# rustformers/llm

Measured on AMD Instinct MI355X. Metric: decode tokens/s LLaMA-7B Q4_0, higher is better.
Workload: dtype i8*i4->i32 block dots, f32 accumulate (W4A8 = ggml's Q4_0·Q8_0)

## Files before the change

### include/ggml_hip.h

```cpp
#ifndef GGML_HIP_H
#define GGML_HIP_H

#include <stdbool.h>
#include <stddef.h>
#include <stdint.h>

#ifdef __cplusplus
extern "C" {
#endif

#define GGML_API __attribute__((visibility("default")))

#define GGML_FILE_MAGIC 0x67676d6c
#define GGML_FILE_VERSION 1
#define GGML_QNT_VERSION 2
#define GGML_QNT_VERSION_FACTOR 1000
#define GGML_MAX_DIMS 4
#define GGML_MAX_NODES 4096
#define GGML_MAX_PARAMS 256
#define GGML_MAX_CONTEXTS 64
#define GGML_MAX_SRC 6
#define GGML_MAX_NAME 48
#define GGML_MAX_OP_PARAMS 32
#define GGML_DEFAULT_N_THREADS 4
// ... 307 lines not shown
GGML_API struct ggml_tensor *ggml_soft_max(struct ggml_context *ctx, struct ggml_tensor *a);
GGML_API struct ggml_tensor *ggml_soft_max_inplace(struct ggml_context *ctx, struct ggml_tensor *a);
GGML_API struct ggml_tensor *ggml_rope(struct ggml_context *ctx, struct ggml_tensor *a, int n_past, int n_dims,
                                       int mode, int n_ctx);
GGML_API struct ggml_tensor *ggml_rope_inplace(struct ggml_context *ctx, struct ggml_tensor *a, int n_past,
                                               int n_dims, int mode, int n_ctx);
GGML_API struct ggml_tensor *ggml_rope_custom_inplace(struct ggml_context *ctx, struct ggml_tensor *a,
                                                      int n_past, int n_dims, int mode, int n_ctx,
                                                      float freq_base, float freq_scale);
GGML_API struct ggml_tensor *ggml_alibi(struct ggml_context *ctx, struct ggml_tensor *a, int n_past, int n_head,
                                        float bias_max);
GGML_API struct ggml_tensor *ggml_flash_attn(struct ggml_context *ctx, struct ggml_tensor *q,
                                             struct ggml_tensor *k, struct ggml_tensor *v, bool masked);
GGML_API struct ggml_tensor *ggml_map_unary_f32(struct ggml_context *ctx, struct ggml_tensor *a,
                                                ggml_unary_op_f32_t fun);
GGML_API struct ggml_tensor *ggml_map_binary_f32(struct ggml_context *ctx, struct ggml_tensor *a,
                                                 struct ggml_tensor *b, ggml_binary_op_f32_t fun);

GGML_API struct ggml_cgraph *ggml_new_graph(struct ggml_context *ctx);
GGML_API size_t ggml_graph_overhead(void);
GGML_API void ggml_build_forward_expand(struct ggml_cgraph *cgraph, struct ggml_tensor *tensor);
GGML_API struct ggml_cgraph ggml_build_forward(struct ggml_tensor *tensor);
GGML_API struct ggml_cplan ggml_graph_plan(struct ggml_cgraph *cgraph, int n_threads);
GGML_API int ggml_graph_compute(struct ggml_cgraph *cgraph, struct ggml_cplan *cplan);
GGML_API void ggml_graph_reset(struct ggml_cgraph *cgraph);

GGML_API size_t ggml_quantize_q4_0(const float *src, void *dst, int n, int k, int64_t *hist);
GGML_API size_t ggml_quantize_q4_1(const float *src, void *dst, int n, int k, int64_t *hist);
GGML_API size_t ggml_quantize_q5_0(const float *src, void *dst, int n, int k, int64_t *hist);
GGML_API size_t ggml_quantize_q5_1(const float *src, void *dst, int n, int k, int64_t *hist);
GGML_API size_t ggml_quantize_q8_0(const float *src, void *dst, int n, int k, int64_t *hist);
GGML_API size_t ggml_quantize_q2_K(const float *src, void *dst, int n, int k, int64_t *hist);
GGML_API size_t ggml_quantize_q3_K(const float *src, void *dst, int n, int k, int64_t *hist);
GGML_API size_t ggml_quantize_q4_K(const float *src, void *dst, int n, int k, int64_t *hist);
GGML_API size_t ggml_quantize_q5_K(const float *src, void *dst, int n, int k, int64_t *hist);
GGML_API size_t ggml_quantize_q6_K(const float *src, void *dst, int n, int k, int64_t *hist);
GGML_API size_t ggml_quantize_chunk(enum ggml_type type, const float *src, void *dst, int start, int n,
                                    int64_t *hist);
GGML_API ggml_type_traits_t ggml_internal_get_type_traits(enum ggml_type i);

GGML_API int ggml_cpu_has_blas(void);
GGML_API int ggml_cpu_has_gpublas(void);

#define GGML_HIP_MAX_DEVICES 16

GGML_API void ggml_init_hipblas(void);
GGML_API void ggml_hip_set_tensor_split(const float *tensor_split);
GGML_API void ggml_hip_mul(const struct ggml_tensor *src0, const struct ggml_tensor *src1,
                           struct ggml_tensor *dst);
GGML_API bool ggml_hip_can_mul_mat(const struct ggml_tensor *src0, const struct ggml_tensor *src1,
                                   struct ggml_tensor *dst);
GGML_API size_t ggml_hip_mul_mat_get_wsize(const struct ggml_tensor *src0, const struct ggml_tensor *src1,
                                           struct ggml_tensor *dst);
GGML_API void ggml_hip_mul_mat(const struct ggml_tensor *src0, const struct ggml_tensor *src1,
                               struct ggml_tensor *dst, void *wdata, size_t wsize);
GGML_API void *ggml_hip_host_malloc(size_t size);
GGML_API void ggml_hip_host_free(void *ptr);
GGML_API void ggml_hip_transform_tensor(void *data, struct ggml_tensor *tensor);
GGML_API void ggml_hip_free_data(struct ggml_tensor *tensor);
GGML_API void ggml_hip_assign_buffers(struct ggml_tensor *tensor);
GGML_API void ggml_hip_assign_buffers_no_scratch(struct ggml_tensor *tensor);
GGML_API void ggml_hip_assign_buffers_force_inplace(struct ggml_tensor *tensor);
GGML_API void ggml_hip_set_main_device(int main_device);
GGML_API void ggml_hip_set_mul_mat_q(bool mul_mat_q);
GGML_API void ggml_hip_set_scratch_size(size_t scratch_size);
GGML_API void ggml_hip_free_scratch(void);
GGML_API bool ggml_hip_compute_forward(struct ggml_compute_params *params, struct ggml_tensor *tensor);

GGML_API void ggml_init_cublas(void);
GGML_API void ggml_cuda_set_tensor_split(const float *tensor_split);
GGML_API void ggml_cuda_mul(const struct ggml_tensor *, const struct ggml_tensor *, struct ggml_tensor *);
GGML_API bool ggml_cuda_can_mul_mat(const struct ggml_tensor *, const struct ggml_tensor *, struct ggml_tensor *);
GGML_API size_t ggml_cuda_mul_mat_get_wsize(const struct ggml_tensor *, const struct ggml_tensor *,
                                            struct ggml_tensor *);
GGML_API void ggml_cuda_mul_mat(const struct ggml_tensor *, const struct ggml_tensor *, struct ggml_tensor *,
                                void *, size_t);
GGML_API void *ggml_cuda_host_malloc(size_t size);
GGML_API void ggml_cuda_host_free(void *ptr);
GGML_API void ggml_cuda_transform_tensor(void *data, struct ggml_tensor *tensor);
GGML_API void ggml_cuda_free_data(struct ggml_tensor *tensor);
GGML_API void ggml_cuda_assign_buffers(struct ggml_tensor *tensor);
GGML_API void ggml_cuda_assign_buffers_no_scratch(struct ggml_tensor *tensor);
GGML_API void ggml_cuda_assign_buffers_force_inplace(struct ggml_tensor *tensor);
GGML_API void ggml_cuda_set_main_device(int main_device);
GGML_API void ggml_cuda_set_mul_mat_q(bool mul_mat_q);
GGML_API void ggml_cuda_set_scratch_size(size_t scratch_size);
GGML_API void ggml_cuda_free_scratch(void);
GGML_API bool ggml_cuda_compute_forward(struct ggml_compute_params *params, struct ggml_tensor *tensor);

GGML_API int ggml_hip_device_count(void);
GGML_API int ggml_hip_slot_physical_device(int slot);
GGML_API int ggml_hip_thread_session_slot(void);
GGML_API int ggml_hip_get_main_device(void);
GGML_API void ggml_hip_bind_thread_device(int device);
GGML_API int ggml_hip_thread_pinned_device(void);
GGML_API void ggml_hip_unbind_thread_device(void);
GGML_API int ggml_hip_get_tensor_split(float *out, int cap);
GGML_API void ggml_hip_set_layer_split(const float *fractions, int n);
GGML_API int ggml_hip_get_layer_split(float *out, int cap);
GGML_API void ggml_hip_copy_between_devices(int dst_device, void *dst, int src_device, const void *src, size_t nbytes);
GGML_API void ggml_hip_synchronize(void);
GGML_API void ggml_hip_tensor_get(const struct ggml_tensor *tensor, void *host_dst, size_t offset, size_t nbytes);
GGML_API void ggml_hip_tensor_set(struct ggml_tensor *tensor, const void *host_src, size_t offset, size_t nbytes);
GGML_API void ggml_hip_memcpy(void *dst, const void *src, size_t nbytes, int kind);
GGML_API void *ggml_hip_tensor_device_ptr(const struct ggml_tensor *tensor);
enum ggml_hip_kclass {
    GGML_HIP_KCLASS_MMVQ = 0,
    GGML_HIP_KCLASS_MMQ_MFMA,
    GGML_HIP_KCLASS_ATTN,
    GGML_HIP_KCLASS_OTHER,
    GGML_HIP_KCLASS_COUNT
};
GGML_API void ggml_hip_timing_begin(void);
GGML_API void ggml_hip_timing_end(void);
GGML_API void ggml_hip_timing_query(int kclass, double *ms, int64_t *launches, double *algo_bytes);
GGML_API void ggml_hip_set_option(const char *key, int value);
GGML_API int ggml_hip_get_option(const char *key);
#define GGML_HIP_KKIND_BASE 16
GGML_API int ggml_hip_bench_plan_class(int kclass, int replays, double *ms_total, int64_t *launches_per_replay,
                                       double *algo_bytes_per_replay);
#define GGML_HIP_COMM_ID_BYTES 128
GGML_API int ggml_hip_comm_unique_id(void *id_out );
GGML_API int ggml_hip_comm_init(int rank, int world, const void *id);
GGML_API void ggml_hip_comm_destroy(void);
GGML_API int ggml_hip_comm_ranks(void);
GGML_API void ggml_hip_comm_send(const void *dev_src, size_t nbytes, int peer);
GGML_API void ggml_hip_comm_recv(void *dev_dst, size_t nbytes, int peer);
GGML_API void ggml_hip_comm_sendrecv(const void *dev_src, int send_peer, void *dev_dst, int recv_peer, size_t nbytes);
GGML_API int ggml_hip_bench_empty(int wgs, int threads, int lds_bytes, int kernarg_bytes, int n_launch, int replays,
                                  double *out);
GGML_API int64_t ggml_hip_get_stat(const char *key);
GGML_API int ggml_hip_graph_compute_begin(struct ggml_cgraph *cgraph);
GGML_API void ggml_hip_graph_compute_end(void);
GGML_API int ggml_hip_graph_prepare(struct ggml_cgraph *cgraph);
GGML_API void ggml_hip_expect_greedy_next(void);
GGML_API int ggml_hip_decode_greedy_chain(struct ggml_cgraph *last, int n, int32_t *out_tokens, float *last_logits);
GGML_API int ggml_hip_decode_batch(struct ggml_cgraph *const *graphs, int n_graphs);
GGML_API int ggml_hip_decode_batch_greedy(struct ggml_cgraph *const *graphs, int n_graphs, int n_steps, int32_t *out_ids);
GGML_API int ggml_hip_topk(const struct ggml_tensor *t, int64_t row, int k, const int32_t *extra_ids, int n_extra,
                           float *out_vals, int32_t *out_ids);
GGML_API int ggml_hip_row_probs(const struct ggml_tensor *logits, int64_t row_begin, int64_t n_rows, const int32_t *targets,
                                float *out_probs);
GGML_API size_t ggml_hip_quantize(enum ggml_type type, const float *src, void *dst, int64_t n, int64_t k, int64_t *hist);
GGML_API int ggml_hip_quantize_resident(const struct ggml_tensor *src, struct ggml_tensor *dst, int64_t *hist);
GGML_API size_t ggml_hip_read_timeline(int64_t *dst, size_t max_records);
GGML_API int ggml_hip_debug_prompt_attention(const float *q, const uint16_t *mem_k, const uint16_t *mem_v, float *out, int N, int E,
                                             int Egqa, int H, int n_past, int64_t C, float scale, int fused);
GGML_API int ggml_hip_debug_prompt_attention_plan(const float *q_raw, const float *q_raw2, const float *rope, const uint16_t *mem_k,
                                                  const uint16_t *mem_v, uint16_t *x16, float *out, int N, int E, int Egqa, int H,
                                                  int n_past, int64_t C, float scale, int f16d);
GGML_API int ggml_hip_debug_exp_le0(uint16_t *out_fast, uint16_t *out_ref);
GGML_API int ggml_hip_debug_token_tail(const float *logits, int V, const float *emb, int E, int n_past, int misalign,
                                       int32_t *id_tail, int32_t *id_argmax, float *slot_logits, float *slot_emb, int32_t *prm_out);
GGML_API int ggml_hip_debug_batch_tail(const float *logits, int B, int V, const int32_t *pos_in, const int32_t *tokens_in,
                                       int32_t *ids_out, int32_t *prm_out, int32_t *pos_out);
GGML_API int ggml_hip_debug_mul_mat_cols(const struct ggml_tensor *w, const float *x, float *out, int N);
GGML_API int ggml_hip_debug_mat_vec_big(const struct ggml_tensor *w0, const struct ggml_tensor *w1, const struct ggml_tensor *w2,
                                        int xsrc, int epi, const float *x, const float *norm_w, float eps, const float *res, float *out,
                                        float *y_out, int n_past, int D, float freq_base, float freq_scale, int64_t C,
                                        uint16_t *mem_k, uint16_t *mem_v);
GGML_API int ggml_hip_debug_mat_vec_kbig(const struct ggml_tensor *w0, const struct ggml_tensor *w1, const struct ggml_tensor *w2,
                                         int xsrc, int epi, const float *x, const float *xw, float eps, const float *res, float *out,
                                         float *y_out, int n_past, int D, float freq_base, float freq_scale, int64_t C,
                                         uint16_t *mem_k, uint16_t *mem_v);
GGML_API int ggml_hip_debug_mat_vec_f16(const struct ggml_tensor *w0, const struct ggml_tensor *w1, const struct ggml_tensor *w2,
                                        int xsrc, int epi, const float *x, const float *xw, float eps, const float *res, float *out,
                                        float *y_out, int n_past, int D, float freq_base, float freq_scale, int64_t C,
                                        uint16_t *mem_k, uint16_t *mem_v, int ncols);
GGML_API int ggml_hip_share_stream(int slot, int with_slot);
GGML_API const char *ggml_hip_version(void);

#ifdef __cplusplus
}
#endif

#ifdef __cplusplus
#define GGML_ABI_ASSERT(c, m) static_assert(c, m)
#else
#define GGML_ABI_ASSERT(c, m) _Static_assert(c, m)
#endif
GGML_ABI_ASSERT(sizeof(struct ggml_object) == 32, "ggml_object size (lib.rs:239)");
GGML_ABI_ASSERT(offsetof(struct ggml_object, type) == 24, "ggml_object.type");
GGML_ABI_ASSERT(sizeof(struct ggml_tensor) == 272, "ggml_tensor size (lib.rs:446)");
GGML_ABI_ASSERT(offsetof(struct ggml_tensor, ne) == 16, "ggml_tensor.ne");
GGML_ABI_ASSERT(offsetof(struct ggml_tensor, nb) == 48, "ggml_tensor.nb");
GGML_ABI_ASSERT(offsetof(struct ggml_tensor, op) == 80, "ggml_tensor.op");
GGML_ABI_ASSERT(offsetof(struct ggml_tensor, op_params) == 84, "ggml_tensor.op_params");
GGML_ABI_ASSERT(offsetof(struct ggml_tensor, is_param) == 116, "ggml_tensor.is_param");
GGML_ABI_ASSERT(offsetof(struct ggml_tensor, grad) == 120, "ggml_tensor.grad");
GGML_ABI_ASSERT(offsetof(struct ggml_tensor, src) == 128, "ggml_tensor.src");
GGML_ABI_ASSERT(offsetof(struct ggml_tensor, perf_runs) == 176, "ggml_tensor.perf_runs");
GGML_ABI_ASSERT(offsetof(struct ggml_tensor, data) == 200, "ggml_tensor.data");
GGML_ABI_ASSERT(offsetof(struct ggml_tensor, name) == 208, "ggml_tensor.name");
GGML_ABI_ASSERT(offsetof(struct ggml_tensor, extra) == 256, "ggml_tensor.extra");
GGML_ABI_ASSERT(offsetof(struct ggml_tensor, padding) == 264, "ggml_tensor.padding");
GGML_ABI_ASSERT(sizeof(struct ggml_cplan) == 16424, "ggml_cplan size");
GGML_ABI_ASSERT(offsetof(struct ggml_cplan, n_tasks) == 20, "ggml_cplan.n_tasks");
GGML_ABI_ASSERT(offsetof(struct ggml_cplan, abort_callback) == 16408, "ggml_cplan.abort_callback");
GGML_ABI_ASSERT(sizeof(struct ggml_cgraph) == 164520, "ggml_cgraph size (lib.rs:651)");
GGML_ABI_ASSERT(offsetof(struct ggml_cgraph, nodes) == 8, "ggml_cgraph.nodes");
GGML_ABI_ASSERT(offsetof(struct ggml_cgraph, leafs) == 65544, "ggml_cgraph.leafs");
GGML_ABI_ASSERT(offsetof(struct ggml_cgraph, visited_hash_table) == 98312, "ggml_cgraph.visited_hash_table");
GGML_ABI_ASSERT(offsetof(struct ggml_cgraph, perf_runs) == 164496, "ggml_cgraph.perf_runs");
GGML_ABI_ASSERT(sizeof(struct ggml_scratch) == 24, "ggml_scratch size");
GGML_ABI_ASSERT(sizeof(struct ggml_init_params) == 24, "ggml_init_params size");
GGML_ABI_ASSERT(sizeof(struct ggml_compute_params) == 32, "ggml_compute_params size");
GGML_ABI_ASSERT(offsetof(struct ggml_compute_params, wsize) == 16, "ggml_compute_params.wsize");
GGML_ABI_ASSERT(sizeof(ggml_type_traits_t) == 40, "ggml_type_traits_t size");

#endif
```

### llm_amd/csrc/backend_state.inc

```

[[noreturn]] void die(const char *fmt, ...) {
    char buf[1024];
    va_list ap;
    va_start(ap, fmt);
    vsnprintf(buf, sizeof(buf), fmt, ap);
    va_end(ap);
    fatal_note("%s", buf);
    abort();
}

int g_cur_slot();
struct Arena {
    uintptr_t base = 0;
    size_t size = 0;
    char *dev = nullptr;
    bool live = true;
    bool is_scratch = false;
};

struct DevTensor {
    uint32_t magic = 0x48495054;
    int slot = (int)(g_cur_slot());
    uintptr_t host = 0;
    size_t nbytes = 0;
    char *dev = nullptr;
    size_t dev_bytes = 0;
    bool soa = false;
    bool auto_uploaded = false;
    int refs = 1;
    bool zero_filled = false;
    uintptr_t owner_hdr = 0;
    QWeight qw{};
    char *w16 = nullptr;
    size_t w16_size = 0;
    bool ksoa = false;
    KWeight kw{};
    ggml_type type = GGML_TYPE_F32;
    int64_t ne[4] = {0, 0, 0, 0};
};

struct Timing {
    bool on = false;
    struct Rec {
        hipEvent_t a, b;
    };
    std::vector<Rec> recs[GGML_HIP_KCLASS_COUNT];
    std::vector<Rec> pool;
    double bytes[GGML_HIP_KCLASS_COUNT] = {0, 0, 0, 0};
    int64_t launches[GGML_HIP_KCLASS_COUNT] = {0, 0, 0, 0};
};

#define GGML_HIP_MAX_BACKENDS 16
struct Backend {
    int slot = 0;
    bool inited = false;
    int device = 0;
    hipStream_t stream = nullptr;
    hipStream_t own_stream = nullptr;
    std::recursive_mutex mu;
    hipEvent_t xfer_ev = nullptr;
    int opt_fuse_heads = 1, opt_attn_one = 1, opt_attn_split = 1;
    std::map<uintptr_t, Arena> arenas;
    std::map<uintptr_t, DevTensor *> tensors;
    std::map<uintptr_t, DevTensor *> auto_tensors;
    struct WsChunk {
        char *p;
        size_t size;
    };
    std::vector<WsChunk> ws_chunks;
    size_t ws_off = 0;
    Timing timing;
    int opt_fuse = 1, opt_plan = 1, opt_plan_k = 1, opt_plan_multi = 1, opt_plan_prompt = 1, opt_graph = 1, opt_big = 1, opt_kbig = 1;
    int opt_chain_k = 0, opt_prepare = 1, opt_plan_batch = 1, opt_plan_f16 = 1, opt_plan_batch_chain = 1;
    int opt_fuse_attn = 1, opt_fuse_wo = 1, opt_warm_mb = 24, opt_affine = 1;
    int opt_act_quant = 0, opt_mmq_i8 = 0;
    int opt_mmq_min = 32, opt_k_prompt_min = 12, opt_mmq_fuse = 3, opt_mmq_cols = 1, opt_mmq_t256 = 1, opt_attn_fused = 1;
    int opt_mmq_w16 = 1, opt_w16_headroom_gb = 16;
    int opt_probe = 0;
    std::atomic<size_t> w16_bytes{0};
    uint64_t w16_gen = 1;
    int num_cus = 256;
    long long *timeline = nullptr;
    size_t timeline_bytes = 0;
    int timeline_wgs = 4;
    uint64_t stat_plan_tokens = 0, stat_generic_graphs = 0, stat_split_tokens = 0, stat_prompt_plan_tokens = 0, stat_fused_tokens = 0, stat_kplan_tokens = 0, stat_fused_heads_tokens = 0, stat_fused_wo_tokens = 0, stat_fused_affine_tokens = 0, stat_prepared_tokens = 0;
    uint64_t stat_alibi_fused = 0;
    uint64_t stat_batch_tokens = 0, stat_batch_steps = 0, stat_batch_chain_steps = 0, stat_batch_chain_tokens = 0;
    uint64_t stat_flash_attn_nodes = 0;
    enum { MMQ_K_PLAIN, MMQ_K_DMA_P8, MMQ_K_W16_P8, MMQ_K_W16_256, MMQ_K_I8, MMQ_K_COUNT };
    uint64_t stat_mmq[MMQ_K_COUNT] = {0, 0, 0, 0, 0};
    void *chain_plan = nullptr;
    ggml_cgraph *chain_graph = nullptr;
    bool pending_wait = false;
    bool pending_light = false;
    int opt_speculate_next = 0, opt_token_tail = 1;
    bool greedy_hint = false;
    struct Spec {
        bool pending = false;
        void *plan = nullptr;
        int n_past = 0, av = 0;
        int parity = 0;
        int32_t fed_id = 0;
        bool fed_id_valid = false;
        int cooldown = 0;
    } spec;
    struct TailWait {
        void *plan = nullptr;
        int q = 0;
        void *logits_dst = nullptr, *emb_dst = nullptr;
        bool staged = false;
    } tail;
    void *res_plan = nullptr;
    uint64_t stat_tail_tokens = 0, stat_result_copies = 0, stat_tail_hits = 0, stat_tail_misses = 0;
    uint64_t stat_spec_hits = 0, stat_spec_misses = 0;
    unsigned *ferr_pin = nullptr;
    void *ferr_plan = nullptr;
    int opt_fused_fallback = 1, opt_fused_rearm_tokens = 256;
    uint64_t fused_rearm_at = 0;
    uint64_t fused_rearm_stretch = 0;
    int fused_saved_fuse_attn = 0, fused_saved_attn_one = 0;
    uint64_t stat_fused_rearms = 0;
    uint64_t stat_cols_warm_launches = 0;
    int opt_test_fused_timeout = 0;
    uint64_t stat_fused_timeouts = 0;
    uint64_t ns_match = 0, ns_launch = 0, ns_wait = 0, ns_compute = 0, ns_mirror = 0, stat_mirror_bytes = 0;
    size_t dead_shadow_bytes = 0;
    uint64_t arena_seen = 0;
    void *prep = nullptr;
    int opt_gen = 0;
    int xcd_labels = -1;
    void *hot_line = nullptr;
    int session_records = 0;
};
enum : unsigned {
    OPT_ENV = 1,
    OPT_DROPS = 2,
    OPT_DEVICE = 4,
    OPT_ACTION = 8,
};
enum OptEffect { FX_NONE, FX_ACT_QUANT, FX_TIMELINE, FX_MMQ_W16, FX_W16_RELEASE, FX_FUSE_ATTN, FX_SPECULATE_NEXT, FX_FUSED_REARM_TOKENS, FX_TEST_FUSED_TIMEOUT, FX_SERIAL_STAGE_SLOTS };
struct OptRow {
    const char *key;
    int Backend::*field;
    unsigned flags;
    OptEffect fx = FX_NONE;
    int lo = 0, hi = -1;
};
static const OptRow g_options[] = {
    {"fuse", &Backend::opt_fuse, OPT_ENV},
    {"plan", &Backend::opt_plan, OPT_ENV},
    {"plan_k", &Backend::opt_plan_k, OPT_ENV | OPT_DROPS},
    {"plan_f16", &Backend::opt_plan_f16, OPT_ENV | OPT_DROPS},
    {"plan_multi", &Backend::opt_plan_multi, OPT_ENV | OPT_DROPS},
    {"plan_prompt", &Backend::opt_plan_prompt, OPT_ENV | OPT_DROPS},
    {"plan_batch", &Backend::opt_plan_batch, OPT_ENV | OPT_DROPS},
    {"plan_batch_chain", &Backend::opt_plan_batch_chain, OPT_ENV},
    {"graph", &Backend::opt_graph, OPT_ENV},
    {"big", &Backend::opt_big, OPT_ENV | OPT_DROPS},
    {"kbig", &Backend::opt_kbig, OPT_ENV | OPT_DROPS},
    {"chain_k", &Backend::opt_chain_k, OPT_ENV, FX_NONE, 0, 64},
    {"prepare", &Backend::opt_prepare, OPT_ENV},
    {"speculate_next", &Backend::opt_speculate_next, OPT_ENV, FX_SPECULATE_NEXT},
    {"token_tail", &Backend::opt_token_tail, OPT_ENV, FX_SPECULATE_NEXT},
    {"fuse_attn", &Backend::opt_fuse_attn, OPT_ENV | OPT_DROPS, FX_FUSE_ATTN},
    {"fuse_wo", &Backend::opt_fuse_wo, OPT_ENV | OPT_DROPS},
    {"warm_mb", &Backend::opt_warm_mb, OPT_ENV | OPT_DROPS},
    {"affine", &Backend::opt_affine, OPT_ENV | OPT_DROPS},
    {"fuse_heads", &Backend::opt_fuse_heads, OPT_ENV | OPT_DROPS},
    {"attn_split", &Backend::opt_attn_split, OPT_ENV | OPT_DROPS},
    {"attn_one", &Backend::opt_attn_one, OPT_ENV | OPT_DROPS},
    {"fused_fallback", &Backend::opt_fused_fallback, OPT_ENV},
    {"fused_rearm_tokens", &Backend::opt_fused_rearm_tokens, OPT_ENV, FX_FUSED_REARM_TOKENS},
    {"act_quant", &Backend::opt_act_quant, OPT_ENV | OPT_DEVICE, FX_ACT_QUANT},
    {"mmq_i8", &Backend::opt_mmq_i8, OPT_ENV},
    {"mmq_min", &Backend::opt_mmq_min, OPT_ENV},
    {"k_prompt_min", &Backend::opt_k_prompt_min, OPT_ENV},
    {"mmq_fuse", &Backend::opt_mmq_fuse, OPT_ENV},
    {"mmq_cols", &Backend::opt_mmq_cols, OPT_ENV | OPT_DROPS},
    {"mmq_t256", &Backend::opt_mmq_t256, OPT_ENV | OPT_DROPS},
    {"attn_fused", &Backend::opt_attn_fused, OPT_ENV},
    {"mmq_w16", &Backend::opt_mmq_w16, OPT_ENV | OPT_DROPS | OPT_DEVICE, FX_MMQ_W16},
    {"w16_headroom_gb", &Backend::opt_w16_headroom_gb, OPT_ENV},
    {"w16_release", nullptr, OPT_DEVICE | OPT_ACTION, FX_W16_RELEASE},
    {"serial_stage_slots", nullptr, 0, FX_SERIAL_STAGE_SLOTS},
    {"timeline", nullptr, OPT_DEVICE, FX_TIMELINE},
    {"probe", &Backend::opt_probe, OPT_DROPS},
    {"test_fused_timeout", &Backend::opt_test_fused_timeout, OPT_DROPS, FX_TEST_FUSED_TIMEOUT},
};
const OptRow &opt_row(const char *key, const char *who) {
    for (const OptRow &o : g_options)
        if (!strcmp(o.key, key)) return o;
    die("%s: unknown key '%s'", who, key);
}
inline int opt_value(const OptRow &o, int v) {
    if (o.fx == FX_ACT_QUANT) return v ? 1 : 0;
    return o.lo <= o.hi ? std::min(o.hi, std::max(o.lo, v)) : v;
}
struct StatRow {
    const char *key;
    uint64_t Backend::*field;
};
static const StatRow g_counters[] = {
    {"plan_tokens", &Backend::stat_plan_tokens},
    {"fused_attn_tokens", &Backend::stat_fused_tokens},
    {"fused_heads_tokens", &Backend::stat_fused_heads_tokens},
    {"fused_wo_tokens", &Backend::stat_fused_wo_tokens},
    {"fused_affine_tokens", &Backend::stat_fused_affine_tokens},
    {"attn_split_tokens", &Backend::stat_split_tokens},
    {"kplan_tokens", &Backend::stat_kplan_tokens},
    {"prepared_tokens", &Backend::stat_prepared_tokens},
    {"prompt_plan_tokens", &Backend::stat_prompt_plan_tokens},
    {"batch_decode_tokens", &Backend::stat_batch_tokens},
    {"batch_decode_steps", &Backend::stat_batch_steps},
    {"batch_chain_steps", &Backend::stat_batch_chain_steps},
    {"batch_chain_tokens", &Backend::stat_batch_chain_tokens},
    {"cols_warm_launches", &Backend::stat_cols_warm_launches},
    {"fused_rearms", &Backend::stat_fused_rearms},
    {"spec_hits", &Backend::stat_spec_hits},
    {"spec_misses", &Backend::stat_spec_misses},
    {"tail_tokens", &Backend::stat_tail_tokens},
    {"tail_hits", &Backend::stat_tail_hits},
    {"tail_misses", &Backend::stat_tail_misses},
    {"result_copies", &Backend::stat_result_copies},
    {"generic_graphs", &Backend::stat_generic_graphs},
    {"alibi_fused", &Backend::stat_alibi_fused},
    {"flash_attn_nodes", &Backend::stat_flash_attn_nodes},
    {"ns_match", &Backend::ns_match},
    {"ns_launch", &Backend::ns_launch},
    {"ns_wait", &Backend::ns_wait},
    {"ns_compute", &Backend::ns_compute},
    {"ns_mirror", &Backend::ns_mirror},
    {"mirror_bytes", &Backend::stat_mirror_bytes},
};
std::recursive_mutex g_mu;
std::map<std::string, int> g_opt_log;
float g_tensor_split[GGML_HIP_MAX_BACKENDS] = {1.0f};
float g_layer_split[GGML_HIP_MAX_BACKENDS] = {0.0f};
int g_layer_split_n = 0;
Backend g_backends[GGML_HIP_MAX_BACKENDS];
std::atomic<int> g_default_slot{0};
std::atomic<int> g_dev_slots[64];
std::atomic<uint64_t> g_dev_gen[64];
std::atomic<uint64_t> g_dev_wgen[64];
thread_local Backend *g_cur = &g_backends[0];
thread_local bool tl_pinned = false;
#define g (*g_cur)
int g_cur_slot() { return (int)(g_cur - g_backends); }
std::atomic<int> g_dev_serial_stages[64];
inline int device_sharers() {
    const int n = g_dev_slots[g.device & 63].load(std::memory_order_relaxed), ser = g_dev_serial_stages[g.device & 63].load(std::memory_order_relaxed);
    return std::max(1, n - (ser > 1 ? std::min(ser, n) - 1 : 0));
}
inline int device_siblings() {
    int n = 0;
    for (int i = 0; i < GGML_HIP_MAX_BACKENDS; i++)
        if (&g_backends[i] != g_cur && g_backends[i].inited && g_backends[i].device == g.device) n++;
    return n;
}
void bind_device();
void sync_arenas();
std::atomic<int> g_calls_inside{0}, g_calls_inside_peak{0};
thread_local int tl_lock_depth = 0;
struct SlotLock {
    Backend *b;
    void enter() {
        b->mu.lock();
        if (tl_lock_depth++ == 0) {
            const int n = g_calls_inside.fetch_add(1, std::memory_order_relaxed) + 1;
            int peak = g_calls_inside_peak.load(std::memory_order_relaxed);
            while (n > peak && !g_calls_inside_peak.compare_exchange_weak(peak, n, std::memory_order_relaxed)) {}
        }
    }
    SlotLock() {
        if (!tl_pinned) g_cur = &g_backends[g_default_slot.load(std::memory_order_relaxed)];
        b = g_cur;
        enter();
        if (b->inited) bind_device();
        sync_arenas();
    }
    explicit SlotLock(Backend *slot) : b(slot) { enter(); }
    ~SlotLock() {
        if (--tl_lock_depth == 0) g_calls_inside.fetch_sub(1, std::memory_order_relaxed);
        b->mu.unlock();
    }
    SlotLock(const SlotLock &) = delete;
    SlotLock &operator=(const SlotLock &) = delete;
};
struct DevOnce {
    bool done[GGML_HIP_MAX_BACKENDS] = {};
    bool first() {
        bool &d = done[g.slot];
        if (d) return false;
        d = true;
        return true;
    }
};
template <auto Kern>
void lds_opt_in(size_t launch_lds, size_t max_bytes) {
    static DevOnce opted;
    if (launch_lds > 64 * 1024 && opted.first())
        HIP_CHECK(hipFuncSetAttribute((const void *)Kern, hipFuncAttributeMaxDynamicSharedMemorySize, (int)max_bytes));
}

int kt_of(ggml_type t) {
    switch (t) {
        case GGML_TYPE_Q2_K: return KT_Q2_K;
        case GGML_TYPE_Q3_K: return KT_Q3_K;
        case GGML_TYPE_Q4_K: return KT_Q4_K;
        case GGML_TYPE_Q5_K: return KT_Q5_K;
        case GGML_TYPE_Q6_K: return KT_Q6_K;
        default: return -1;
    }
}
int qt_of(ggml_type t) {
    switch (t) {
        case GGML_TYPE_Q4_0: return QT_Q4_0;
        case GGML_TYPE_Q4_1: return QT_Q4_1;
        case GGML_TYPE_Q5_0: return QT_Q5_0;
        case GGML_TYPE_Q5_1: return QT_Q5_1;
        case GGML_TYPE_Q8_0: return QT_Q8_0;
        default: return -1;
    }
}
#define CT(x) (decltype(x)::value)
template <class F>
void with_qt(int qt, F &&f, const char *bad = nullptr) {
    if (bad && (qt < QT_Q4_0 || qt > QT_Q8_0)) die("%s", bad);
    switch (qt) {
        case QT_Q4_0: f(std::integral_constant<int, QT_Q4_0>{}); break;
        case QT_Q4_1: f(std::integral_constant<int, QT_Q4_1>{}); break;
        case QT_Q5_0: f(std::integral_constant<int, QT_Q5_0>{}); break;
        case QT_Q5_1: f(std::integral_constant<int, QT_Q5_1>{}); break;
        default: f(std::integral_constant<int, QT_Q8_0>{}); break;
    }
}
template <class F>
void with_kt(int kt, F &&f) {
    switch (kt) {
        case KT_Q4_K: f(std::integral_constant<int, KT_Q4_K>{}); break;
        case KT_Q6_K: f(std::integral_constant<int, KT_Q6_K>{}); break;
        case KT_Q2_K: f(std::integral_constant<int, KT_Q2_K>{}); break;
        case KT_Q3_K: f(std::integral_constant<int, KT_Q3_K>{}); break;
        default: f(std::integral_constant<int, KT_Q5_K>{}); break;
    }
}
template <class F>
void with_bool(bool b, F &&f) {
    if (b)
        f(std::true_type{});
    else
        f(std::false_type{});
}
static inline bool qt_f16d(int qt) { return qt == QT_Q4_0 || qt == QT_Q5_0 || qt == QT_Q8_0; }

thread_local int tl_device = -1;
void bind_device() {
    if (tl_device != g.device) {
        HIP_CHECK(hipSetDevice(g.device));
        tl_device = g.device;
    }
}
int slot_count() {
    int n = 0;
    if (hipGetDeviceCount(&n) != hipSuccess) return 0;
    if (const char *v = getenv("GGML_HIP_VIRTUAL_DEVICES")) n = std::max(n, atoi(v));
    if (const char *v = getenv("GGML_HIP_SESSION_SLOTS")) n = std::max(n, atoi(v));
    return std::min(n, GGML_HIP_MAX_BACKENDS);
}
thread_local int tl_auto_slot = -1;
int g_session_threads[GGML_HIP_MAX_BACKENDS] = {};
inline int session_slots_env() {
    static const int n = getenv("GGML_HIP_SESSION_SLOTS") ? atoi(getenv("GGML_HIP_SESSION_SLOTS")) : 0;
    return n;
}
inline int slot_physical_device(int slot) {
// ... 439 lines not shown
```

### llm_amd/csrc/backend_tools.inc

```
namespace {
template <int NARG>
struct EmptyArgs {
    long long *ts;
    int idx;
    int pad[(NARG - 12) / 4];
};
template <int NARG>
__global__ void __launch_bounds__(1024) k_empty(const EmptyArgs<NARG> a, int last_arg) {
    extern __shared__ __attribute__((aligned(16))) char smem[];
    long long t0;
    asm volatile("s_memrealtime %0\n\ts_waitcnt lgkmcnt(0)" : "=s"(t0));
    const int v = a.pad[(NARG - 12) / 4 - 1] + last_arg;
    long long t1 = v != 0x7fffffff ? (long long)wall_clock64() : 0;
    if (v == 0x12345678) smem[threadIdx.x] = 1;
    if (threadIdx.x == 0 && blockIdx.x == 0) {
        a.ts[a.idx * 4] = t0;
        a.ts[a.idx * 4 + 1] = t1;
        a.ts[a.idx * 4 + 2] = (long long)wall_clock64();
    }
}
template <int NARG>
void empty_launch(int wgs, int threads, int lds, long long *ts, int idx) {
    EmptyArgs<NARG> a;
    memset(&a, 0, sizeof(a));
// ... 358 lines not shown
        if (!t || t->type != GGML_TYPE_F16 || t->ne[0] != K || t->ne[2] != 1 || t->ne[3] != 1 || !ggml_is_contiguous(t)) return -1;
        Ms[i] = t->ne[1];
    }
    if (K % 8 != 0) return -1;
    if (epi == KE_QKV && (!mem_k || !mem_v || D < 2 || D % 2 || D > 256 || Ms[0] % D || Ms[1] % D || Ms[1] != Ms[2] || n_past < 0 ||
                          n_past + ncols > C))
        return -1;
    std::vector<char *> owned;
    debug_hot_line();
    F16W fw[3];
    for (int i = 0; i < nw; i++) {
        const ggml_tensor *t = ts[i];
        DevTensor *e = extra_of(t);
        if (!e) e = find_tensor((uintptr_t)t->data);
        const char *d = e && !e->soa && !e->ksoa ? e->dev + ((uintptr_t)t->data - e->host) : debug_buf(ggml_nbytes(t), t->data, owned);
        fw[i] = F16W{(const __half *)d, (int64_t)t->nb[1] / 2, Ms[i]};
    }
    if (!f16_launch_ok(nw, fw, K, xsrc, epi)) {
        for (char *b : owned) HIP_CHECK(hipFree(b));
        return -1;
    }
    const size_t nx = (size_t)ncols * K * 4;
    char *dx = debug_buf(nx, x, owned);
    char *dxw = xw ? debug_buf(xsrc == KX_SILU_MUL ? nx : (size_t)K * 4, xw, owned) : nullptr;
    char *dres = res ? debug_buf((size_t)ncols * Ms[0] * 4, res, owned) : nullptr;
    const int64_t Mrow = epi == KE_ROW ? Ms[0] + Ms[1] + Ms[2] : Ms[0];
    const size_t n_out = (size_t)ncols * Mrow * 4;
    char *dout = debug_buf(n_out, nullptr, owned);
    char *dy = (xsrc == KX_NORM && y_out) ? debug_buf(nx, nullptr, owned) : nullptr;
    const RowSrc src{xsrc, (const float *)dx, (const float *)dxw, eps, epi == KE_ROW ? (float *)dy : nullptr};
    char *dk = nullptr, *dv = nullptr;
    const size_t nkv = epi == KE_QKV ? (size_t)C * Ms[1] * 2 : 0;
    if (epi == KE_QKV) {
        DecParams hp;
        memset(&hp, 0, sizeof(hp));
        hp.n_past = n_past;
        DecParams *prm = (DecParams *)debug_buf(sizeof(DecParams), &hp, owned);
        float *rope = (float *)debug_buf((size_t)ncols * 128 * 4, nullptr, owned);
        hipLaunchKernelGGL(k_rope_table, dim3((unsigned)ncols), dim3(128), 0, g.stream, (const DecParams *)prm, powf(freq_base, -2.0f / (float)D),
                           freq_scale, D >> 1, rope, (unsigned *)nullptr);
        HIP_CHECK(hipGetLastError());
        dk = debug_buf(nkv, mem_k, owned);
        dv = debug_buf(nkv, mem_v, owned);
        F16Qkv qa;
        memset(&qa, 0, sizeof(qa));
        qa.rope = rope; qa.prm = prm; qa.mem_k = (__half *)dk; qa.mem_v = (__half *)dv; qa.Egqa = Ms[1]; qa.C = C; qa.D = D;
        float *ds3[3] = {(float *)dout, nullptr, nullptr};
        const int kinds[3] = {0, 1, 2};
        launch_f16(3, fw, ds3, K, src, nullptr, ncols, KE_QKV, &qa, kinds);
    } else if (epi == KE_GATE) {
        float *ds2[2] = {(float *)dout, nullptr};
        launch_f16(2, fw, ds2, K, src, nullptr, ncols, KE_GATE);
    } else if (nw == 1) {
        float *ds1[1] = {(float *)dout};
        launch_f16(1, fw, ds1, K, src, (const float *)dres, ncols);
    } else {
        float *ds[3] = {nullptr, nullptr, nullptr};
        for (int i = 0; i < nw; i++) ds[i] = (float *)debug_buf((size_t)ncols * Ms[i] * 4, nullptr, owned);
        launch_f16(nw, fw, ds, K, src, nullptr, ncols);
        int64_t at = 0;
        for (int i = 0; i < nw; i++) {
            HIP_CHECK(hipMemcpy2DAsync(dout + at * 4, (size_t)Mrow * 4, ds[i], (size_t)Ms[i] * 4, (size_t)Ms[i] * 4, (size_t)ncols, hipMemcpyDeviceToDevice, g.stream));
            at += Ms[i];
        }
    }
    if (dy && epi != KE_ROW) {
        float *ds1[1] = {(float *)debug_buf((size_t)ncols * Ms[0] * 4, nullptr, owned)};
        launch_f16(1, fw, ds1, K, RowSrc{KX_NORM, (const float *)dx, (const float *)dxw, eps, (float *)dy}, nullptr, ncols);
    }
    d2h_queue(out, dout, n_out + DEBUG_GUARD);
    if (dy) d2h_queue(y_out, dy, nx + DEBUG_GUARD);
    if (dk) {
        d2h_queue(mem_k, dk, nkv + DEBUG_GUARD);
        d2h_queue(mem_v, dv, nkv + DEBUG_GUARD);
    }
    d2h_finish();
    for (char *b : owned) HIP_CHECK(hipFree(b));
    return 0;
}

int ggml_hip_debug_prompt_attention_plan(const float *q_raw, const float *q_raw2, const float *rope, const uint16_t *mem_k,
                                         const uint16_t *mem_v, uint16_t *x16, float *out, int N, int E, int Egqa, int H, int n_past,
                                         int64_t C, float scale, int f16d) {
    SlotLock lk;
    ensure_init();
    finish_pending();
    if (!q_raw || !rope || !mem_k || !mem_v || !x16 || N < 1 || H < 1 || E % H || n_past < 0) return -1;
    const int64_t D = E / H, T = (int64_t)n_past + N;
    if (Egqa < D || Egqa % D || H % (Egqa / D) || T > C || C % 8 || !prompt_attn_fits(D, T)) return -1;
    const int64_t Hkv = Egqa / D;
    std::vector<char *> owned;
    const size_t nq = (size_t)N * E * 4, nkv = (size_t)C * Egqa * 2, nx = (size_t)N * E * 2;
    char *dq = debug_buf(nq * (q_raw2 ? 2 : 1), nullptr, owned);
    h2d_bulk(dq, q_raw, nq);
    if (q_raw2) h2d_bulk(dq + nq, q_raw2, nq);
    char *dr = debug_buf((size_t)N * 128 * 4, rope, owned);
    char *dk = debug_buf(nkv, mem_k, owned), *dv = debug_buf(nkv, mem_v, owned);
    char *dx = debug_buf(nx, nullptr, owned), *dout = debug_buf(nq, nullptr, owned);
    prompt_attention(true, (const float *)dq, (const __half *)dk, (const __half *)dv, (float *)dout, nullptr, nullptr, N, E, Egqa, H, Hkv,
                     D, n_past, C, scale, (_Float16 *)dx, f16d != 0, (const float *)dr, q_raw2 ? (int64_t)N * E : 0);
    d2h_queue(x16, dx, nx + DEBUG_GUARD);
    if (out) d2h_queue(out, dout, nq + DEBUG_GUARD);
    d2h_finish();
    for (char *b : owned) HIP_CHECK(hipFree(b));
    return 0;
}

__global__ void __launch_bounds__(256) k_debug_exp_le0(uint16_t *out_fast, uint16_t *out_ref) {
    const unsigned i = blockIdx.x * 256 + threadIdx.x;
    const float x = __half2float(__ushort_as_half((unsigned short)i));
    out_fast[i] = __half_as_ushort(__float2half_rn(exp_le0(x)));
    out_ref[i] = __half_as_ushort(__float2half_rn(expf(x)));
}
int ggml_hip_debug_exp_le0(uint16_t *out_fast, uint16_t *out_ref) {
    SlotLock lk;
    ensure_init();
    finish_pending();
    uint16_t *d;
    dev_malloc((void **)&d, 2 * 65536 * 2, "debug exp");
    hipLaunchKernelGGL(k_debug_exp_le0, dim3(256), dim3(256), 0, g.stream, d, d + 65536);
    HIP_CHECK(hipGetLastError());
    HIP_CHECK(hipStreamSynchronize(g.stream));
    HIP_CHECK(hipMemcpy(out_fast, d, 65536 * 2, hipMemcpyDeviceToHost));
    HIP_CHECK(hipMemcpy(out_ref, d + 65536, 65536 * 2, hipMemcpyDeviceToHost));
    HIP_CHECK(hipFree(d));
    return 0;
}

int ggml_hip_debug_token_tail(const float *logits, int V, const float *emb, int E, int n_past, int misalign, int32_t *id_tail,
                              int32_t *id_argmax, float *slot_logits, float *slot_emb, int32_t *prm_out) {
    if (!logits || V < 1 || (emb && E < 1) || misalign < 0 || misalign > 3 || !id_tail || !id_argmax || !slot_logits || !prm_out) return -1;
    SlotLock lk;
    ensure_init();
    finish_pending();
    const size_t lb = ((size_t)(V + 4) * 4 + 255) & ~(size_t)255, eb = ((size_t)(std::max(E, 1) + 4) * 4 + 255) & ~(size_t)255;
    const size_t emb_off = ((size_t)V * 4 + 255) & ~(size_t)255, id_off = emb_off + eb;
    char *d = nullptr, *slot = nullptr;
    dev_malloc((void **)&d, lb + eb + 1024, "debug token tail");
    HIP_CHECK(hipHostMalloc((void **)&slot, id_off + 256, hipHostMallocDefault));
    memset(slot, 0xff, id_off + 256);
    float *dl = (float *)d + misalign, *de = (float *)(d + lb) + misalign;
    DecParams *pa = (DecParams *)(d + lb + eb), *pb = pa + 1;
    int *ida = (int *)(pb + 1);
    DecParams hp;
    memset(&hp, 0, sizeof(hp));
    hp.n_past = n_past;
    HIP_CHECK(hipStreamSynchronize(g.stream));
    HIP_CHECK(hipMemcpy(dl, logits, (size_t)V * 4, hipMemcpyHostToDevice));
    if (emb) HIP_CHECK(hipMemcpy(de, emb, (size_t)E * 4, hipMemcpyHostToDevice));
    HIP_CHECK(hipMemcpy(pa, &hp, sizeof(hp), hipMemcpyHostToDevice));
    HIP_CHECK(hipMemcpy(pb, &hp, sizeof(hp), hipMemcpyHostToDevice));
    hipLaunchKernelGGL(k_argmax_next, dim3(1), dim3(1024), 0, g.stream, (const float *)dl, V, pa, ida);
    hipLaunchKernelGGL(k_token_tail, dim3(TOKEN_TAIL_WGS), dim3(1024), 0, g.stream, (const float *)dl, V, emb ? (const float *)de : (const float *)nullptr,
                       E, pb, slot, (int)emb_off, (int)id_off);
    HIP_CHECK(hipGetLastError());
    HIP_CHECK(hipStreamSynchronize(g.stream));
    HIP_CHECK(hipMemcpy(id_argmax, ida, 4, hipMemcpyDeviceToHost));
    HIP_CHECK(hipMemcpy(&hp, pb, sizeof(hp), hipMemcpyDeviceToHost));
    prm_out[0] = hp.n_past;
    prm_out[1] = hp.token;
    prm_out[2] = hp.tokens[0];
    *id_tail = *(const int32_t *)(slot + id_off);
    memcpy(slot_logits, slot, (size_t)V * 4);
    if (emb && slot_emb) memcpy(slot_emb, slot + emb_off, (size_t)E * 4);
    HIP_CHECK(hipHostFree(slot));
    HIP_CHECK(hipFree(d));
    return 0;
}

int ggml_hip_decode_greedy_chain(struct ggml_cgraph *last, int n, int32_t *out_tokens, float *last_logits) {
    SlotLock lk;
    return decode_greedy_chain(last, n, out_tokens, last_logits);
}

int ggml_hip_decode_batch(struct ggml_cgraph *const *graphs, int n_graphs) {
    if (!graphs || n_graphs < 2 || n_graphs > BATCH_COLS_MAX) return -1;
    for (int i = 0; i < n_graphs; i++)
        if (!graphs[i]) return -1;
    SlotLock lk;
    const uint64_t t0 = now_ns();
    const int r = decode_batch(graphs, n_graphs);
    g.ns_compute += now_ns() - t0;
    return r;
}

int ggml_hip_decode_batch_greedy(struct ggml_cgraph *const *graphs, int n_graphs, int n_steps, int32_t *out_ids) {
    if (!graphs || n_graphs < 2 || n_graphs > BATCH_COLS_MAX || n_steps < 1 || n_steps > BATCH_CHAIN_MAX_STEPS) return -1;
    if (n_steps > 1 && !out_ids) return -1;
    for (int i = 0; i < n_graphs; i++)
        if (!graphs[i]) return -1;
    SlotLock lk;
    const uint64_t t0 = now_ns();
    const int r = decode_batch_steps(graphs, n_graphs, n_steps, out_ids, true);
    g.ns_compute += now_ns() - t0;
    return r;
}

int ggml_hip_debug_batch_tail(const float *logits, int B, int V, const int32_t *pos_in, const int32_t *tokens_in, int32_t *ids_out,
                              int32_t *prm_out, int32_t *pos_out) {
    if (!logits || B < 1 || B > BATCH_COLS_MAX || V < 1 || !pos_in || !tokens_in || !ids_out || !prm_out || !pos_out) return -1;
    SlotLock lk;
    ensure_init();
    finish_pending();
    const size_t lb = ((size_t)B * V * 4 + 255) & ~(size_t)255;
    char *d = nullptr;
    dev_malloc((void **)&d, lb + 1024, "debug batch tail");
    DecParams *dp = (DecParams *)(d + lb);
    BatchCols *db = (BatchCols *)(d + lb + 256);
    int *dids = (int *)(d + lb + 768);
    static_assert(sizeof(DecParams) <= 256 && sizeof(BatchCols) <= 512 && BATCH_COLS_MAX * 4 <= 256, "debug batch tail: layout");
    DecParams hp;
    BatchCols hb;
    memset(&hp, 0, sizeof(hp));
    memset(&hb, 0, sizeof(hb));
    for (int i = 0; i < 32; i++) hp.tokens[i] = tokens_in[i];
    for (int i = 0; i < BATCH_COLS_MAX; i++) hb.pos[i] = pos_in[i];
    hp.n_past = pos_in[0];
    hp.token = tokens_in[0];
    HIP_CHECK(hipStreamSynchronize(g.stream));
    HIP_CHECK(hipMemcpy(d, logits, (size_t)B * V * 4, hipMemcpyHostToDevice));
    HIP_CHECK(hipMemcpy(dp, &hp, sizeof(hp), hipMemcpyHostToDevice));
    HIP_CHECK(hipMemcpy(db, &hb, sizeof(hb), hipMemcpyHostToDevice));
    HIP_CHECK(hipMemset(dids, 0xff, BATCH_COLS_MAX * 4));
    hipLaunchKernelGGL(k_batch_argmax_next, dim3((unsigned)B), dim3(1024), 0, g.stream, (const float *)d, V, dp, db, dids);
    HIP_CHECK(hipGetLastError());
    HIP_CHECK(hipStreamSynchronize(g.stream));
    HIP_CHECK(hipMemcpy(ids_out, dids, (size_t)B * 4, hipMemcpyDeviceToHost));
    HIP_CHECK(hipMemcpy(&hp, dp, sizeof(hp), hipMemcpyDeviceToHost));
    HIP_CHECK(hipMemcpy(&hb, db, sizeof(hb), hipMemcpyDeviceToHost));
    prm_out[0] = hp.n_past;
    prm_out[1] = hp.token;
    for (int i = 0; i < 32; i++) prm_out[2 + i] = hp.tokens[i];
    for (int i = 0; i < BATCH_COLS_MAX; i++) pos_out[i] = hb.pos[i];
    HIP_CHECK(hipFree(d));
    return 0;
}

int64_t ggml_hip_get_stat(const char *key) {
    SlotLock lk;
    for (const StatRow &c : g_counters)
        if (!strcmp(c.key, key)) return (int64_t)(g.*c.field);
    const std::string k(key);
    if (k == "w16_bytes") return (int64_t)g.w16_bytes;
    if (k.rfind("mmq_launches_", 0) == 0) {
        static const char *names[Backend::MMQ_K_COUNT] = {"plain", "dma_p8", "w16_p8", "w16_256", "i8"};
        for (int i = 0; i < Backend::MMQ_K_COUNT; i++)
            if (k.substr(13) == names[i]) return (int64_t)g.stat_mmq[i];
        return -1;
    }
    if (k == "graph_replays") {
        int64_t n = 0;
        for (auto *p : g_plans) n += (int64_t)p->replays;
        return n;
    }
    if (k == "plans") return (int64_t)g_plans.size();
    if (k == "num_cus") {
        ensure_init();
        return (int64_t)g.num_cus;
    }
    if (k == "fused_attn_timeouts") {
        int64_t n = (int64_t)g.stat_fused_timeouts;
        if (g.inited) HIP_CHECK(hipStreamSynchronize(g.stream));
        if (g.ferr_pin) n += *(volatile unsigned *)g.ferr_pin;
        return n;
    }
    if (k == "peak_concurrent_calls") return (int64_t)g_calls_inside_peak.load();
    return -1;
}
size_t ggml_hip_read_timeline(int64_t *dst, size_t max_records) {
    SlotLock lk;
    if (!g.timeline) return 0;
    const size_t n = std::min(max_records, g.timeline_bytes / 64);
    HIP_CHECK(hipStreamSynchronize(g.stream));
    HIP_CHECK(hipMemcpy(dst, g.timeline, n * 64, hipMemcpyDeviceToHost));
    return n;
}
const char *ggml_hip_version(void) { return "libggml_hip 0.1 (gfx950)"; }

}
```

### llm_amd/csrc/kernels/decode.h

```cpp
#pragma once
#include "common.h"
#include "mmvq.h"
#include "ops.h"

struct DecParams {
    int n_past;
    int token;
    int store_at;
    int pad1;
    int tokens[32];
};
constexpr int BATCH_COLS_MAX = 8;
struct BatchCols {
    int pos[BATCH_COLS_MAX];
    __half *mem_k[BATCH_COLS_MAX];
    __half *mem_v[BATCH_COLS_MAX];
};

__device__ __forceinline__ int argmax_first_block(const float *__restrict__ logits, int V) {
    __shared__ float s_v[16];
    __shared__ int s_i[16];
    const int tid = threadIdx.x, lane = tid & 63, wave = tid >> 6;
    float bv = -INFINITY;
    int bi = 0x7fffffff;
    for (int i0 = tid; i0 < V; i0 += 8 * 1024) {
        float v8[8];
#pragma unroll
        for (int u = 0; u < 8; u++) {
            const int i = i0 + u * 1024;
            v8[u] = i < V ? logits[i] : -INFINITY;
        }
#pragma unroll
        for (int u = 0; u < 8; u++) {
            const int i = i0 + u * 1024;
            if (i < V && (v8[u] > bv || bi == 0x7fffffff)) {
                bv = v8[u];
                bi = i;
            }
        }
    }
    auto better = [](float v, int i, float bv_, int bi_) { return v > bv_ || (v == bv_ && i < bi_); };
#pragma unroll
    for (int off = 32; off >= 1; off >>= 1) {
        const float ov = __shfl_xor(bv, off);
        const int oi = __shfl_xor(bi, off);
        if (better(ov, oi, bv, bi)) {
            bv = ov;
            bi = oi;
        }
    }
    if (lane == 0) {
        s_v[wave] = bv;
        s_i[wave] = bi;
    }
    __syncthreads();
    if (tid == 0) {
        for (int w = 1; w < 16; w++)
            if (better(s_v[w], s_i[w], bv, bi)) {
                bv = s_v[w];
                bi = s_i[w];
            }
    }
    return bi;
}
__global__ void __launch_bounds__(1024) k_argmax_next(const float *__restrict__ logits, int V, DecParams *prm,
                                                      int *__restrict__ out) {
    const int bi = argmax_first_block(logits, V);
    if (threadIdx.x == 0) {
        prm->token = bi;
        prm->tokens[0] = bi;
        prm->n_past = prm->n_past + 1;
        out[0] = bi;
    }
}
__global__ void __launch_bounds__(1024) k_batch_argmax_next(const float *__restrict__ logits, int V, DecParams *prm, BatchCols *bc,
                                                            int *__restrict__ out) {
    const int c = blockIdx.x;
    if (c >= BATCH_COLS_MAX) return;
    const int bi = argmax_first_block(logits + (size_t)c * V, V);
    if (threadIdx.x == 0) {
        const int pos = bc->pos[c] + 1;
        prm->tokens[c] = bi;
        bc->pos[c] = pos;
        out[c] = bi;
        if (c == 0) {
            prm->token = bi;
            prm->n_past = pos;
        }
    }
}
__global__ void __launch_bounds__(256) k_kv_row_save(const DecParams *__restrict__ prm, const __half *__restrict__ mem_k,
                                                     const __half *__restrict__ mem_v, __half *__restrict__ save, int L, int C, int Egqa) {
    const int pos = prm->n_past;
    if (pos < 0 || pos >= C) return;
    const long n = (long)L * Egqa;
    for (long i = (long)blockIdx.x * 256 + threadIdx.x; i < n; i += (long)gridDim.x * 256) {
        const long il = i / Egqa, c = i % Egqa;
        save[i] = mem_k[(il * C + pos) * Egqa + c];
        save[n + i] = mem_v[(il * Egqa + c) * C + pos];
    }
}
__global__ void __launch_bounds__(256) k_kv_row_restore(int pos, __half *__restrict__ mem_k, __half *__restrict__ mem_v,
                                                        const __half *__restrict__ save, int L, int C, int Egqa) {
    if (pos < 0 || pos >= C) return;
    const long n = (long)L * Egqa;
    for (long i = (long)blockIdx.x * 256 + threadIdx.x; i < n; i += (long)gridDim.x * 256) {
        const long il = i / Egqa, c = i % Egqa;
        mem_k[(il * C + pos) * Egqa + c] = save[i];
        mem_v[(il * Egqa + c) * C + pos] = save[n + i];
    }
}
constexpr int TOKEN_TAIL_WGS = 8;
__global__ void __launch_bounds__(1024) k_token_tail(const float *__restrict__ logits, int V, const float *__restrict__ emb, int E,
                                                     DecParams *prm, char *__restrict__ slot, int emb_off, int id_off) {
    const int gtid = blockIdx.x * 1024 + threadIdx.x, total = gridDim.x * 1024;
    float *sl = (float *)slot, *se = (float *)(slot + emb_off);
    if (((uintptr_t)logits & 15) == 0) {
        const int V4 = V >> 2;
        for (int i = gtid; i < V4; i += total) ((float4 *)sl)[i] = ((const float4 *)logits)[i];
        if (gtid < (V & 3)) sl[(V4 << 2) + gtid] = logits[(V4 << 2) + gtid];
    } else {
        for (int i = gtid; i < V; i += total) sl[i] = logits[i];
    }
    if (emb) {
        if (((uintptr_t)emb & 15) == 0 && (E & 3) == 0)
            for (int i = gtid; i < (E >> 2); i += total) ((float4 *)se)[i] = ((const float4 *)emb)[i];
        else
            for (int i = gtid; i < E; i += total) se[i] = emb[i];
    }
    if (blockIdx.x != 0) return;
    const int bi = argmax_first_block(logits, V);
    if (threadIdx.x == 0) {
        prm->token = bi;
        prm->tokens[0] = bi;
        prm->n_past = prm->n_past + 1;
        *(int *)(slot + id_off) = bi;
    }
}

__device__ __forceinline__ void rope_table_pair(int pos, int c, int kk, float theta_scale, float freq_scale, float *__restrict__ out) {
    float theta = freq_scale * (float)pos;
    for (int t = 0; t < kk; t++) theta *= theta_scale;
    out[c * 128 + 2 * kk] = cosf(theta);
    out[c * 128 + 2 * kk + 1] = sinf(theta);
}
__global__ void __launch_bounds__(128) k_rope_table(const DecParams *__restrict__ prm, float theta_scale, float freq_scale,
                                                    int half_d, float *__restrict__ out, unsigned *epoch = nullptr) {
    const int kk = threadIdx.x, c = blockIdx.x;
    if (epoch && kk == 0 && c == 0) {
        const unsigned e = *epoch + 1u;
        *epoch = e ? e : 1u;
    }
    if (kk >= half_d) return;
    rope_table_pair(prm->n_past + c, c, kk, theta_scale, freq_scale, out);
}
__global__ void __launch_bounds__(128) k_rope_table_batch(const BatchCols *__restrict__ bc, float theta_scale, float freq_scale,
                                                          int half_d, float *__restrict__ out) {
    const int kk = threadIdx.x, c = blockIdx.x;
    if (kk >= half_d) return;
    rope_table_pair(bc->pos[c], c, kk, theta_scale, freq_scale, out);
}

template <bool F16_D>
__device__ __forceinline__ void rmsnorm_quant_body(const float *__restrict__ x, const float *__restrict__ w, float eps, int E,
                                                   float *y_f32 , int8_t *lo, int8_t *hi, float *dq, int *sumq,
                                                   float *dT ,
                                                   int *sT ) {
    extern __shared__ __attribute__((aligned(16))) char smem[];
    float *s_y = (float *)smem;
    __shared__ double s_part[16];
    const int tid = threadIdx.x;
    {
        const int64_t r = blockIdx.x;
        x += r * E;
        if (y_f32) y_f32 += r * E;
        lo += r * (E / 2);
        hi += r * (E / 2);
        dq += r * (E / 32);
        sumq += r * (E / 32);
    }
    constexpr int PT = 8;
    const bool in_regs = E <= PT * 1024;
    float xv[PT], wv[PT];
    if (in_regs) {
#pragma unroll
        for (int k = 0; k < PT; k++) {
            const int i = tid + k * 1024;
            xv[k] = i < E ? x[i] : 0.0f;
            wv[k] = i < E ? w[i] : 0.0f;
        }
    }
    double s = 0.0;
    if (in_regs) {
#pragma unroll
        for (int k = 0; k < PT; k++)
            if (tid + k * 1024 < E) s += (double)(xv[k] * xv[k]);
    } else {
        for (int i = tid; i < E; i += 1024) {
            const float v = x[i];
            s += (double)(v * v);
        }
    }
    s = wave_sum_f64(s);
    if ((tid & 63) == 0) s_part[tid >> 6] = s;
    __syncthreads();
    double tot = 0.0;
#pragma unroll
    for (int i = 0; i < 16; i++) tot += s_part[i];
    const float mean = (float)(tot / (double)E);
    const float scale = 1.0f / sqrtf(mean + eps);
    if (in_regs) {
#pragma unroll
        for (int k = 0; k < PT; k++) {
            const int i = tid + k * 1024;
            if (i < E) {
                const float v = (xv[k] * scale) * wv[k];
                s_y[i] = v;
                if (y_f32) y_f32[i] = v;
            }
        }
    } else {
        for (int i = tid; i < E; i += 1024) {
            const float v = (x[i] * scale) * w[i];
            s_y[i] = v;
            if (y_f32) y_f32[i] = v;
        }
    }
    __syncthreads();
    const int nblk = E / 32, l = tid & 31;
    for (int b = tid >> 5; b < nblk; b += 32) {
        const float v = s_y[b * 32 + l];
        float amax = fabsf(v);
        amax = g32_max_f32(amax);
        const float d = amax / 127.0f;
        const float id = act_id(amax, d, aq_scalar());
        const int q = act_q(v * id, aq_scalar());
        int sq = q;
        sq = g32_sum_i32(sq);
        (l < 16 ? lo : hi)[b * 16 + (l & 15)] = (int8_t)q;
        if (l == 0) {
            dq[b] = F16_D ? round_f16(d) : d;
            sumq[b] = sq;
            if (dT) {
                const int64_t o = (int64_t)(blockIdx.x >> 3) * nblk * 8 + b * 8 + (blockIdx.x & 7);
                dT[o] = F16_D ? round_f16(d) : d;
                sT[o] = sq;
            }
        }
    }
}
template <bool F16_D>
__global__ void __launch_bounds__(1024) k_rmsnorm_quant(const float *__restrict__ x, const float *__restrict__ w, float eps, int E,
                                                        float *y_f32, int8_t *lo, int8_t *hi, float *dq, int *sumq,
                                                        float *dT = nullptr, int *sT = nullptr) {
    rmsnorm_quant_body<F16_D>(x, w, eps, E, y_f32, lo, hi, dq, sumq, dT, sT);
}

constexpr int CW_MAX = 12;
struct ColsWarm {
    const uint8_t *base[CW_MAX];
    uint32_t row_bytes[CW_MAX];
    int row0[CW_MAX], rows[CW_MAX];
    int n;
    int G, gq, gr;
    int wg;
};
__device__ __forceinline__ void cols_warm(const ColsWarm &cw, const int first , unsigned *junk) {
    typedef const __attribute__((address_space(1))) void *wg_ptr;
    typedef __attribute__((address_space(3))) void *wl_ptr;
    const int b = (int)blockIdx.x, x = b & 7, tid = (int)threadIdx.x;
    const int b0 = first + ((x - first) & 7);
    const int j = (b - b0) >> 3, nj = ((int)gridDim.x - b0 + 7) >> 3;
    for (int c = x + 8 * j; c < cw.G; c += 8 * nj) {
        const int g0 = c * cw.gq + (c < cw.gr ? c : cw.gr), nlg = cw.gq + (c < cw.gr ? 1 : 0);
        const int R0 = 16 * g0, R1 = 16 * (g0 + (nlg < cw.wg ? nlg : cw.wg));
        for (int a = 0; a < cw.n; a++) {
            const int lo_r = (R0 > cw.row0[a] ? R0 : cw.row0[a]) - cw.row0[a];
            const int hi_r = (R1 < cw.row0[a] + cw.rows[a] ? R1 : cw.row0[a] + cw.rows[a]) - cw.row0[a];
            if (lo_r >= hi_r) continue;
            const uint8_t *p = cw.base[a] + (size_t)lo_r * cw.row_bytes[a];
            const uint32_t bytes = (uint32_t)(hi_r - lo_r) * cw.row_bytes[a];
            for (uint32_t off = (uint32_t)tid << 7; off < bytes; off += 1024u << 7)
                __builtin_amdgcn_global_load_lds((wg_ptr)(p + off), (wl_ptr)junk, 4, 0, 0);
        }
    }
}
template <bool F16_D>
__global__ void __launch_bounds__(1024) k_rmsnorm_quant_warm(const float *__restrict__ x, const float *__restrict__ w, float eps, int E,
// ... 501 lines not shown
```

### llm_amd/csrc/plan_build.inc

```
static DevTensor *plan_rec(const ggml_tensor *t) {
    DevTensor *e = extra_of(t);
    if (!e) e = find_tensor((uintptr_t)t->data);
    return e;
}
static KWeight plan_kw(const ggml_tensor *t) {
    DevTensor *e = plan_rec(t);
    if (!e || !e->ksoa || (uintptr_t)t->data != e->host) die("decode plan: K-quant weight '%s' has no resident planar copy", t->name);
    return e->kw;
}
static QWeight plan_qw(const ggml_tensor *t) {
    DevTensor *e = plan_rec(t);
    if (!e || !e->soa || (uintptr_t)t->data != e->host) die("decode plan: weight '%s' has no resident SoA copy", t->name);
    return e->qw;
}
static F16W plan_f16w(const ggml_tensor *t) {
    DevTensor *e = plan_rec(t);
    if (!e || e->soa || e->ksoa) die("decode plan: F16 weight '%s' has no resident copy", t->name);
    return F16W{(const __half *)(e->dev + ((uintptr_t)t->data - e->host)), (int64_t)t->nb[1] / 2, t->ne[1]};
}
static uint64_t rec_id(const ggml_tensor *t) {
    DevTensor *e = plan_rec(t);
    return e ? (uint64_t)(uintptr_t)e->dev : 0;
}

static bool plan_weights_resident(const LlamaMatch &m) {
    auto ok_q = [](const ggml_tensor *t) {
        DevTensor *e = plan_rec(t);
        if (t->type == GGML_TYPE_F16) return e && !e->soa && !e->ksoa && f16_weight_ok(plan_f16w(t));
        return e && (e->soa || e->ksoa) && (uintptr_t)t->data == e->host;
    };
    auto ok_raw = [](const ggml_tensor *t) {
        DevTensor *e = plan_rec(t);
        return e && !e->soa;
    };
    if (!ok_raw(m.memory_k) || !ok_raw(m.memory_v)) return false;
    if (m.wte && !ok_q(m.wte)) return false;
    if (m.output && (!ok_q(m.output) || !ok_raw(m.norm))) return false;
    if (m.stage_in && !ok_raw(m.stage_in)) return false;
    if (m.stage_out && !ok_raw(m.stage_out)) return false;
    for (auto &l : m.layers) {
        for (int i = 0; i < LAYER_MATS; i++)
            if (!ok_q(l.at(i))) return false;
        if (!ok_raw(l.attn_norm) || !ok_raw(l.ffn_norm)) return false;
    }
    return true;
}

static std::vector<uint64_t> plan_signature(const LlamaMatch &m, bool session = true) {
    std::vector<uint64_t> s;
    auto f2u = [](float f) { uint32_t u; memcpy(&u, &f, 4); return (uint64_t)u; };
    s.push_back((uint64_t)m.N);
    for (uint64_t v : {(uint64_t)m.L, (uint64_t)m.E, (uint64_t)m.H, (uint64_t)m.Hkv, (uint64_t)m.D, (uint64_t)m.F,
                       (uint64_t)m.V, (uint64_t)m.C, (uint64_t)m.n_dims, (uint64_t)m.wtype, f2u(m.eps),
                       f2u(m.freq_base), f2u(m.freq_scale), f2u(m.kq_scale)})
        s.push_back(v);
    for (const ggml_tensor *t : {m.wte, m.norm, m.output, m.stage_in, m.stage_out}) s.push_back(t ? rec_id(t) : 0);
    if (session)
        for (const ggml_tensor *t : {m.memory_k, m.memory_v}) s.push_back(rec_id(t));
    for (auto &l : m.layers) {
        for (const ggml_tensor *t : {l.attn_norm, l.ffn_norm}) s.push_back(rec_id(t));
        for (int i = 0; i < LAYER_MATS; i++) s.push_back(rec_id(l.at(i)));
    }
    if (m.f16w) {
        auto rec = [&](const ggml_tensor *t) {
            if (!t) return;
            s.push_back((uint64_t)(uintptr_t)t->data);
            s.push_back((uint64_t)t->nb[1]);
            s.push_back((uint64_t)t->ne[1]);
        };
        rec(m.wte);
        rec(m.output);
        for (auto &l : m.layers)
            for (int i = 0; i < LAYER_MATS; i++) rec(l.at(i));
    }
    if (!session) return s;
    s.push_back(m.logits ? (uint64_t)(uintptr_t)dev_ptr(m.logits) : 0);
    s.push_back(m.embedding ? (uint64_t)(uintptr_t)dev_ptr(m.embedding) : 0);
    return s;
}
static std::vector<const ggml_tensor *> plan_matrices(const LlamaMatch &m) {
    std::vector<const ggml_tensor *> ws;
    for (auto &l : m.layers)
        for (int i = 0; i < LAYER_MATS; i++) ws.push_back(l.at(i));
    if (m.output) ws.push_back(m.output);
    return ws;
}
static size_t w16_need(const std::vector<const ggml_tensor *> &ws) {
    size_t need = 0;
    for (auto *w : ws) {
        DevTensor *e = plan_rec(w);
        if (e && !e->w16) need += e->ksoa ? (size_t)e->kw.M * (size_t)e->kw.nsb * 512 : (size_t)e->qw.M * e->qw.nb * 64;
    }
    return need;
}
template <class W, class F>
static std::vector<LayerMats<W>> plan_layer_weights(const LlamaMatch &m, F &&of) {
    std::vector<LayerMats<W>> v(m.layers.size());
    for (size_t il = 0; il < v.size(); il++)
        for (int i = 0; i < LAYER_MATS; i++) v[il].at(i) = of(m.layers[il].at(i));
    return v;
}
static bool k_prompt_weights(const LlamaMatch &m, DecodePlan *p) {
    const std::vector<const ggml_tensor *> ws = plan_matrices(m);
    for (auto *w : ws) {
        DevTensor *e = plan_rec(w);
        if (!e || !e->ksoa || (uintptr_t)w->data != e->host) return false;
    }
    if (const size_t need = w16_need(ws)) {
        size_t free_b = 0, total_b = 0;
        if (hipMemGetInfo(&free_b, &total_b) != hipSuccess || free_b < need + ((size_t)1 << 30) + w16_headroom()) return false;
        for (auto *w : ws)
            if (!ensure_w16_k(plan_rec(w))) return false;
    }
    if (!p) return true;
    auto qw_of = [&](const ggml_tensor *t) {
        DevTensor *e = plan_rec(t);
        QWeight w;
        memset(&w, 0, sizeof(w));
        w.M = e->kw.M;
        w.nb = e->kw.nsb * 8;
        w.qt = QT_Q8_0;
        w.w16 = e->w16;
        return w;
    };
    p->lw = plan_layer_weights<QWeight>(m, qw_of);
    if (m.output) p->output = qw_of(m.output);
    p->w16_gen = g.w16_gen;
    return true;
}
static void xcd_labels_probe() {
    if (g.xcd_labels >= 0) return;
    g.xcd_labels = 0;
    if (g.num_cus % 8 != 0 || g.num_cus < 16) return;
    unsigned *d = nullptr;
    dev_malloc((void **)&d, (size_t)g.num_cus * 4, "XCD probe");
    std::vector<unsigned> id((size_t)g.num_cus);
    bool ok = true;
    for (int rep = 0; rep < 2 && ok; rep++) {
        hipLaunchKernelGGL(k_xcc_ids, dim3((unsigned)g.num_cus), dim3(1024), 0, g.stream, d);
        HIP_CHECK(hipMemcpyAsync(id.data(), d, id.size() * 4, hipMemcpyDeviceToHost, g.stream));
        HIP_CHECK(hipStreamSynchronize(g.stream));
        unsigned seen = 0;
        for (int b = 0; b < 8; b++) seen |= 1u << id[(size_t)b];
        ok = __builtin_popcount(seen) == 8;
        for (int b = 8; b < g.num_cus && ok; b++) ok = id[(size_t)b] == id[(size_t)(b & 7)];
    }
    HIP_CHECK(hipFree(d));
    g.xcd_labels = ok ? 1 : 0;
}
struct PoolCarver {
    char *base;
    size_t off = 0;
    template <class T>
    void take(T *&field, size_t bytes) {
        if (base && bytes) field = (T *)(base + off);
        off = (off + bytes + 255) & ~(size_t)255;
    }
};
static void plan_pool_layout(DecodePlan *p, PoolCarver &c) {
    const LlamaMatch &m = p->m;
    const size_t R = (size_t)m.N;
    const size_t E = (size_t)m.E, F = (size_t)m.F, S = (size_t)p->att_S;
    const bool one = m.N == 1, spec = one && m.logits, multi = m.N >= 2 && !m.prompt, kq = m.kquant;
    const size_t Lg = one ? (size_t)m.L : 1;
    c.take(p->att_sc, (size_t)m.H * m.C * 4);
    c.take(p->att_pmax, (size_t)m.H * S * 4);
    c.take(p->att_part, (size_t)m.H * S * m.D * 4);
    c.take(p->att_mxg, Lg * m.H * S * 8);
    c.take(p->att_sumg, Lg * m.H * S * 16);
    c.take(p->att_partg, one ? Lg * m.H * S * m.D * 8 : 0);
    c.take(p->att_cnt, (size_t)m.H * 4);
    c.take(p->hot, 256);
    c.take(p->logits_alt, spec ? (size_t)m.V * 4 : 0);
    c.take(p->emb_alt, spec ? E * 4 : 0);
    c.take(p->kv_save[0], spec ? (size_t)m.L * m.Egqa * 4 : 0);
    c.take(p->kv_save[1], spec ? (size_t)m.L * m.Egqa * 4 : 0);
    c.take(p->epoch, 256);
    const size_t units = (size_t)((m.E + 2 * m.Egqa) / 2);
    c.take(p->gran, one ? (size_t)m.L * units * 8 : 0);
    c.take(p->dead_gran, one ? units * 8 : 0);
    c.take(p->ogran, one ? (size_t)m.L * (size_t)(m.E / 32) * OGRAN * 8 : 0);
    c.take(p->bcols, p->batch ? sizeof(BatchCols) : 0);
    c.take(p->logits_out, p->batch ? R * m.V * 4 : 0);
    c.take(p->emb_out, p->batch ? R * E * 4 : 0);
    c.take(p->prm, sizeof(DecParams));
    c.take(p->rope, std::max<size_t>(8, R) * 128 * 4);
    c.take(p->xa, R * E * 4);
    c.take(p->xb, R * E * 4);
    c.take(p->q, R * E * 4);
    c.take(p->gate, R * F * 4);
    c.take(p->e_lo, R * E / 2);
    c.take(p->e_hi, R * E / 2);
    c.take(p->e_d, R * E / 32 * 4);
    c.take(p->e_s, R * E / 32 * 4);
    c.take(p->f_lo, R * F / 2);
    c.take(p->f_hi, R * F / 2);
    c.take(p->f_d, R * F / 32 * 4);
    c.take(p->f_s, R * F / 32 * 4);
    const size_t passes = (R + 7) / 8;
    c.take(p->e_dT, multi ? passes * E / 32 * 32 : 0);
    c.take(p->e_sT, multi ? passes * E / 32 * 32 : 0);
    c.take(p->f_dT, multi ? passes * F / 32 * 32 : 0);
    c.take(p->f_sT, multi ? passes * F / 32 * 32 : 0);
    const size_t kW = std::max(E, F);
    c.take(p->k_kf, kq ? R * m.Egqa * 4 : 0);
    c.take(p->k_vf, kq ? R * m.Egqa * 4 : 0);
    c.take(p->k_att, kq || m.f16w ? R * E * 4 : 0);
    c.take(p->k_g3, kq ? R * F * 4 : 0);
    c.take(p->k_q8, kq ? R * kW : 0);
    c.take(p->k_d8, kq ? R * kW / 256 * 4 : 0);
    c.take(p->k_bs, kq ? R * kW / 256 * 32 : 0);
    c.take(p->p_tok, m.prompt ? R * 4 : 0);
}
static DecodePlan *build_plan(const LlamaMatch &m, std::vector<uint64_t> sig, bool batch = false) {
    if (m.prompt && !m.kquant) {
        const std::vector<const ggml_tensor *> ws = plan_matrices(m);
        size_t free_b = 0, total_b = 0;
        const bool room = hipMemGetInfo(&free_b, &total_b) == hipSuccess && free_b >= w16_need(ws) + w16_headroom();
        if (room)
            for (auto *w : ws) ensure_w16(plan_rec(w));
    }
    xcd_labels_probe();
    if (!g.hot_line) {
        dev_malloc(&g.hot_line, 256, "the dummy ring steps' line");
        HIP_CHECK(hipMemsetAsync(g.hot_line, 0, 256, g.stream));
    }
    DecodePlan *p = new DecodePlan();
    p->sig = std::move(sig);
    p->m = m;
    if (m.wte) (m.f16w ? (void)(p->f_wte = plan_f16w(m.wte)) : m.kquant ? (void)(p->k_wte = plan_kw(m.wte)) : (void)(p->wte = plan_qw(m.wte)));
    if (m.output) {
        if (m.f16w) p->f_output = plan_f16w(m.output);
        else if (m.kquant) p->k_output = plan_kw(m.output);
        else p->output = plan_qw(m.output);
        p->norm = (const float *)dev_ptr(m.norm);
    }
    if (m.stage_in) p->stage_in = (float *)dev_ptr(m.stage_in);
    if (m.stage_out) p->stage_out = (float *)dev_ptr(m.stage_out);
    p->batch = batch;
    if (!batch) {
        p->mem_k = (__half *)dev_ptr(m.memory_k);
        p->mem_v = (__half *)dev_ptr(m.memory_v);
    }
    if (m.f16w) p->flw = plan_layer_weights<F16W>(m, plan_f16w);
    else if (m.kquant) p->klw = plan_layer_weights<KWeight>(m, plan_kw);
    else p->lw = plan_layer_weights<QWeight>(m, plan_qw);
    for (auto &l : m.layers) p->ln.push_back({(const float *)dev_ptr(l.attn_norm), (const float *)dev_ptr(l.ffn_norm)});
    if (m.embedding && !batch) p->emb_out = (float *)dev_ptr(m.embedding);
    if (m.logits && !batch) p->logits_out = dev_ptr(m.logits);
    p->att_S = plan_att_S(m.H);
    PoolCarver sizes{nullptr};
    plan_pool_layout(p, sizes);
    dev_malloc((void **)&p->pool, sizes.off, "a decode plan's activation pool");
    HIP_CHECK(hipMemsetAsync(p->pool, 0, sizes.off, g.stream));
    PoolCarver carve{p->pool};
    plan_pool_layout(p, carve);
    if (!g.ferr_pin) {
        HIP_CHECK(hipHostMalloc((void **)&g.ferr_pin, 64, hipHostMallocDefault));
        *g.ferr_pin = 0;
    }
    p->ferr = g.ferr_pin;
    return p;
}
```

### llm_amd/csrc/plan_decode.inc

```
struct PlanStats {
    double bytes[GGML_HIP_KCLASS_COUNT] = {0, 0, 0, 0};
    int64_t launches[GGML_HIP_KCLASS_COUNT] = {0, 0, 0, 0};
};
struct LaunchCtx {
    unsigned mask = ~0u, kind_mask = ~0u;
    PlanStats *st = nullptr;
    int ts_idx = 0;
    bool want(int k, double bytes) {
        if (!(mask & (1u << k))) return false;
        if (st) {
            st->bytes[k] += bytes;
            st->launches[k]++;
        }
        return true;
    }
    long long *next_ts() {
        if (!g.timeline) return nullptr;
        if ((size_t)(ts_idx + 1) * g.timeline_wgs * 8 * 8 > g.timeline_bytes) return nullptr;
        return g.timeline + (size_t)(ts_idx++) * g.timeline_wgs * 8;
    }
    template <class F>
    void mmvq(int kind, double bytes, F &&launch) {
        if (!(kind_mask & (1u << kind)) || !want(GGML_HIP_KCLASS_MMVQ, bytes)) return;
        Timed tm(GGML_HIP_KCLASS_MMVQ, bytes);
// ... 42 lines not shown
static void launch_qkv_attn_wo(const BigArgs &ba, const FusedAttnArgs &fa, const WoTailArgs &wt, const FusedShape &sh, size_t lds) {
    const bool two = (wt.w.nb + 63) / 64 <= 2;
    with_bool(two, [&](auto TWO) {
        constexpr int STEPS = CT(TWO) ? 2 : 4;
        lds_opt_in<k_qkv_attn_wo<QT, STEPS>>(lds, ATTN_DECODE_LDS_MAX);
        hipLaunchKernelGGL((k_qkv_attn_wo<QT, STEPS>), dim3(sh.G), dim3(1024), lds, g.stream, ba, fa, wt);
    });
}
static void launch_attn_decode(const DecodePlan *p, int il, int N, int64_t rows, bool f16d, float *out_f32, long long *ts,
                               float *dT = nullptr, int *sT = nullptr) {
    const LlamaMatch &m = p->m;
    with_bool(f16d, [&](auto F16D) {
        lds_opt_in<k_attn_decode<CT(F16D)>>(attn_decode_lds(rows, m.D), ATTN_DECODE_LDS_MAX);
        hipLaunchKernelGGL(k_attn_decode<CT(F16D)>, dim3((unsigned)m.H, (unsigned)N), dim3(1024), attn_decode_lds(rows, m.D), g.stream,
                           (const float *)p->q, (const __half *)p->mem_k_at(il), (const __half *)p->mem_v_at(il), (const DecParams *)p->prm,
                           m.kq_scale, (int)m.D, (int)(m.H / m.Hkv), m.Egqa, m.C, out_f32, p->e_lo, p->e_hi, p->e_d, p->e_s, ts, (int)m.H,
                           rows, dT, sT);
    });
    HIP_CHECK(hipGetLastError());
}
static FusedAttnArgs fused_attn_args(const DecodePlan *p, int il, int S, int64_t Clds) {
    const LlamaMatch &m = p->m;
    FusedAttnArgs fa;
    memset(&fa, 0, sizeof(fa));
    fa.mem_k = p->mem_k_at(il); fa.mem_v = p->mem_v_at(il); fa.prm = p->prm; fa.epoch = p->epoch; fa.gran = p->gran_at(il);
    fa.k_pair0 = (int)(m.E / 2); fa.v_pair0 = (int)((m.E + m.Egqa) / 2);
    fa.scale = m.kq_scale; fa.D = (int)m.D; fa.n_rep = (int)(m.H / m.Hkv); fa.n_head = (int)m.H;
    fa.Egqa = m.Egqa; fa.C = m.C; fa.Clds = Clds;
    fa.err = p->ferr; fa.S = S; fa.layer = il;
    return fa;
}
static AttnSplitOneArgs split_attn_args(const DecodePlan *p, int il) {
    const LlamaMatch &m = p->m;
    AttnSplitOneArgs oa;
    memset(&oa, 0, sizeof(oa));
    AttnSplitArgs &sa = oa.a;
    sa.q = p->q; sa.mem_k = p->mem_k_at(il); sa.mem_v = p->mem_v_at(il); sa.prm = p->prm; sa.scale = m.kq_scale; sa.D = (int)m.D;
    sa.n_rep = (int)(m.H / m.Hkv); sa.n_head = (int)m.H; sa.S = p->att_S; sa.Egqa = m.Egqa; sa.C = m.C;
    sa.lo = p->e_lo; sa.hi = p->e_hi; sa.dq = p->e_d; sa.sumq = p->e_s;
    oa.mx_g = p->att_mxg_at(il); oa.sum_g = p->att_sumg_at(il); oa.part_g = p->att_partg_at(il); oa.cnt = p->att_cnt; oa.epoch = p->epoch; oa.layer = il;
    oa.err = p->ferr;
    return oa;
}
static void launch_attn_split_one(const DecodePlan *p, const AttnSplitOneArgs &oa, bool f16d) {
    const dim3 grid((unsigned)p->m.H, (unsigned)oa.a.S);
    with_bool(f16d, [&](auto F16D) {
        hipLaunchKernelGGL(k_attn_split_one<CT(F16D)>, grid, dim3(1024), attn_split_chunk_max(p->m.C, oa.a.S) * 6, g.stream, oa);
    });
}
template <class F>
static void for_each_weight_array(int qt, const QWeight &q, int64_t nb, F &&f) {
    f((const void *)q.qs, (size_t)nb * 16);
    if (qt == QT_Q8_0) f((const void *)q.qs2, (size_t)nb * 16);
    if (qt == QT_Q5_0 || qt == QT_Q5_1) f((const void *)q.qh, (size_t)nb * 4);
    f((const void *)q.d, (size_t)nb * 2);
    if (qt == QT_Q4_1 || qt == QT_Q5_1) f((const void *)q.m, (size_t)nb * 2);
}
template <class F>
static void for_each_type_run(const KWeight *const *ws, int n, F &&f) {
    for (int i = 0; i < n;) {
        int j = i + 1;
        while (j < n && ws[j]->kt == ws[i]->kt) j++;
        f(i, j);
        i = j;
    }
}
struct ResultDst {
    float *emb;
    char *logits;
};
static ResultDst plan_result_dst(const DecodePlan *p) { return ResultDst{p->res_emb(p->out_set), p->res_logits(p->out_set)}; }
template <class F>
static void plan_open_rows(DecodePlan *p, LaunchCtx &cx, bool batch, double embed_bytes, F &&embed) {
    const LlamaMatch &m = p->m;
    const int N = m.N;
    const float theta_scale = powf(m.freq_base, -2.0f / m.n_dims);
    if (!m.wte) {
        if (cx.want(GGML_HIP_KCLASS_OTHER, (double)N * m.E * 8.0))
            HIP_CHECK(hipMemcpyAsync(p->xa, p->stage_in, (size_t)N * m.E * 4, hipMemcpyDeviceToDevice, g.stream));
    } else {
        cx.other((double)N * m.E * embed_bytes, embed);
    }
    cx.other((double)N * m.D * 4.0, [&] {
        if (batch)
            hipLaunchKernelGGL(k_rope_table_batch, dim3((unsigned)N), dim3(128), 0, g.stream, (const BatchCols *)p->bcols, theta_scale, m.freq_scale,
                               (int)(m.D >> 1), p->rope);
        else
            hipLaunchKernelGGL(k_rope_table, dim3((unsigned)N), dim3(128), 0, g.stream, (const DecParams *)p->prm, theta_scale, m.freq_scale,
                               (int)(m.D >> 1), p->rope, p->epoch);
    });
}
static void launch_attn_decode_batch(const DecodePlan *p, int il, int N, bool f16d, float *out_f32);
static void plan_attn_f32(DecodePlan *p, LaunchCtx &cx, int il, bool long_ctx, bool batch) {
    const LlamaMatch &m = p->m;
    const int N = m.N;
    const double bytes = (double)N * ((double)(m.n_past + N) * m.Egqa * 4.0 + m.E * 9.0);
    if (!cx.want(GGML_HIP_KCLASS_ATTN, bytes)) return;
    Timed tm(GGML_HIP_KCLASS_ATTN, bytes);
    if (batch)
        launch_attn_decode_batch(p, il, N, true, p->k_att);
    else if (long_ctx) {
        AttnSplitOneArgs oa = split_attn_args(p, il);
        oa.out_f32 = p->k_att;
        launch_attn_split_one(p, oa, true);
    } else
        launch_attn_decode(p, il, N, m.C, true, p->k_att, nullptr);
    HIP_CHECK(hipGetLastError());
}
static bool plan_hand_on(DecodePlan *p, LaunchCtx &cx) {
    const LlamaMatch &m = p->m;
    if (m.output) return false;
    if (cx.want(GGML_HIP_KCLASS_OTHER, (double)m.N * m.E * 8.0))
        HIP_CHECK(hipMemcpyAsync(p->stage_out, p->xa, (size_t)m.N * m.E * 4, hipMemcpyDeviceToDevice, g.stream));
    return true;
}

static void plan_launch_all(DecodePlan *p, int av, LaunchCtx cx) {
    const bool long_ctx = av == AV_SPLIT;
    const LlamaMatch &m = p->m;
    const int qt = qt_of(m.wtype);
    const bool f16d = qt_f16d(qt);
    const bool big = g.opt_big != 0;
    const bool fuse_x = big;
    const int64_t E = m.E, F = m.F, nbE = E / 32, nbF = F / 32;
    const QAct actE{(const i32x4 *)p->e_lo, (const i32x4 *)p->e_hi, p->e_d, p->e_s};
    const QAct actF{(const i32x4 *)p->f_lo, (const i32x4 *)p->f_hi, p->f_d, p->f_s};
    const float theta_scale = powf(m.freq_base, -2.0f / m.n_dims);
    const double bb = (double)blk_bytes(qt);
    auto rmsq = [&](const float *x, const float *w, float *y) {
        cx.other((double)E * 9.25, [&] {
            with_bool(f16d, [&](auto F16D) {
                hipLaunchKernelGGL(k_rmsnorm_quant<CT(F16D)>, dim3(1), dim3(1024), (size_t)E * 4, g.stream, x, w, m.eps, (int)E, y,
                                   p->e_lo, p->e_hi, p->e_d, p->e_s);
            });
        });
    };
    auto matvec = [&](int kind, auto EPI, auto XSRC, auto XDEC, const DecMmvqArgs &a, float *y_out, const float *rope, int nwg, double bytes) {
        cx.mmvq(kind, bytes, [&] {
            with_qt(qt, [&](auto QT) {
                if (big)
                    launch_big<CT(QT), CT(EPI), CT(XSRC)>(BigArgs{a, y_out, cx.next_ts(), g.timeline_wgs, rope, g.opt_probe, nullptr, nullptr, 0, p->hot});
                else
                    fuse_x ? launch_dec<CT(QT), CT(EPI), CT(XDEC)>(a, nwg) : launch_dec<CT(QT), CT(EPI), XSRC_Q8>(a, nwg);
            });
        });
    };
    constexpr std::integral_constant<int, EPI_QKV> epi_qkv{};
    constexpr std::integral_constant<int, EPI_ADD> epi_add{};
    constexpr std::integral_constant<int, EPI_GATE> epi_gate{};
    constexpr std::integral_constant<int, EPI_STORE> epi_store{};
    constexpr std::integral_constant<int, XSRC_NORM> x_norm{};
    constexpr std::integral_constant<int, XSRC_Q8> x_q8{};
    constexpr std::integral_constant<int, XSRC_F32> x_f32{};
    if (m.wte)
        cx.other((double)E * 4.6, [&] {
            hipLaunchKernelGGL(k_get_rows_q, dim3((unsigned)((nbE + 255) / 256), 1), dim3(256), 0, g.stream, p->wte,
                               (const int *)&p->prm->token, p->xa, E);
        });
    const FusedShape fsh = long_ctx ? FusedShape{} : fused_qkv_shape(m, av_heads_split(av));
    const bool rope_for_fused = fsh.ok && (cx.mask & (1u << GGML_HIP_KCLASS_MMVQ)) && (cx.kind_mask & 1u) && !(cx.mask & (1u << GGML_HIP_KCLASS_OTHER));
    if (big && (cx.want(GGML_HIP_KCLASS_OTHER, (double)m.D * 4.0) || rope_for_fused)) {
        hipLaunchKernelGGL(k_rope_table, dim3(1), dim3(128), 0, g.stream, (const DecParams *)p->prm, theta_scale,
                           m.freq_scale, (int)(m.D >> 1), p->rope, p->epoch);
        HIP_CHECK(hipGetLastError());
    }
    static const bool same_layer = getenv("GGML_HIP_BENCH_SAME_LAYER") && atoi(getenv("GGML_HIP_BENCH_SAME_LAYER"));
    const bool fuse_wo = fsh.ok && fsh.wo && p->ogran != nullptr;
    const double wo_bytes = (double)E * nbE * bb + nbE * 40.0 + E * 8.0;
    for (int il = 0; il < m.L; il++) {
        const int wl = (same_layer && cx.kind_mask != ~0u) ? 0 : il;
        const DecodePlan::LW &w = p->lw[wl];
        const DecodePlan::LayerNorms &ln = p->ln[wl];
        float *const xin = (il == 0 && !m.wte) ? p->stage_in : p->xa;
        float *const xout = (il == m.L - 1 && !m.output) ? p->stage_out : p->xa;
        if (!fuse_x) rmsq(xin, ln.attn_norm, nullptr);
        {
            DecMmvqArgs a;
            memset(&a, 0, sizeof(a));
            a.w[0] = w.wq; a.w[1] = w.wk; a.w[2] = w.wv;
            a.wg_begin[0] = 0;
            a.wg_begin[1] = (int)((E + 7) / 8);
            a.wg_begin[2] = a.wg_begin[1] + (int)((m.Egqa + 7) / 8);
            const int nwg = a.wg_begin[2] + (int)((m.Egqa + 7) / 8);
            a.x = actE; a.xf = xin; a.xw = ln.attn_norm; a.eps = m.eps;
            a.nb = nbE; a.dst = p->q; a.prm = p->prm; a.mem_k = p->mem_k_at(il); a.mem_v = p->mem_v_at(il);
            a.Egqa = m.Egqa; a.C = m.C; a.D = (int)m.D; a.theta_scale = theta_scale; a.freq_scale = m.freq_scale;
            const double qkv_bytes = (double)(E + 2 * m.Egqa) * nbE * bb + nbE * 40.0 + (E + 2 * m.Egqa) * 4.0;
            if (fsh.ok) {
                const double att_bytes = (double)(m.n_past + 1) * m.Egqa * 4.0 + m.E * 9.0;
                cx.mmvq(0, qkv_bytes + att_bytes + (fuse_wo ? wo_bytes : 0.0), [&] {
                    BigArgs ba{a, nullptr, cx.next_ts(), g.timeline_wgs, p->rope, g.opt_probe, p->gran_at(il), p->epoch, fsh.W, p->hot};
                    FusedAttnArgs fa = fused_attn_args(p, il, fsh.S, attn_decode_rows(m.C, 1, m.H));
                    if (fsh.affine) {
                        ba.aff_hpl = (int)(m.H / 8);
                        ba.aff_shift = m.D == 128 ? 6 : m.D == 64 ? 5 : 4;
                        fa.local_rows = 1;
                    }
                    fa.lo = p->e_lo; fa.hi = p->e_hi; fa.dq = p->e_d; fa.sumq = p->e_s;
                    fa.ts = cx.next_ts(); fa.ts_heads = g.timeline_wgs;
                    fa.mx_g = p->att_mxg_at(il); fa.sum_g = p->att_sumg_at(il); fa.part_g = p->att_partg_at(il); fa.cnt = p->att_cnt;
                    if (g.opt_test_fused_timeout && il == 0) fa.gran = p->dead_gran;
                    const size_t lds = std::max(attn_decode_lds(fa.Clds, m.D), (size_t)((nbE + 63) / 64 * 64) * 40);
                    if (!fuse_wo) {
                        with_qt(qt, [&](auto QT) { launch_qkv_attn<CT(QT)>(ba, fa, fsh, lds); });
                        return;
                    }
                    fa.ogran = p->ogran + (size_t)il * (size_t)(nbE * OGRAN);
                    WoTailArgs wt;
                    memset(&wt, 0, sizeof(wt));
                    wt.w = w.wo; wt.res = xin; wt.dst = p->xb;
                    wt.ts = cx.next_ts(); wt.ts_wgs = g.timeline_wgs;
                    if (g.opt_warm_mb > 0 && big && (cx.kind_mask & 5u) == 5u && g.num_cus % 8 == 0 && F >= (int64_t)g.num_cus * BIG_W) {
                        NextWarm &nw = wt.warm;
                        int64_t wrows = (int64_t)((double)g.opt_warm_mb * 1e6 / (2.0 * (double)nbE * bb)) & ~(int64_t)7;
                        wrows = std::min<int64_t>(wrows, F);
                        for (const QWeight *q : {&w.w1, &w.w3})
                            for_each_weight_array(qt, *q, nbE, [&](const void *b, size_t rb) {
                                if (b && nw.n < WARM_MAX) { nw.base[nw.n] = (const uint8_t *)b; nw.row_bytes[nw.n] = (uint32_t)rb; nw.rows_of[nw.n++] = (int)wrows; }
                            });
                        nw.rows = (int)wrows;
                        nw.bcast = (const uint8_t *)ln.ffn_norm; nw.bcast_bytes = (int)(E * 4);
                        wt.warm_wave = 15;
                    }
                    with_qt(qt, [&](auto QT) { launch_qkv_attn_wo<CT(QT)>(ba, fa, wt, fsh, lds); });
                });
            } else
                matvec(0, epi_qkv, x_norm, x_norm, a, nullptr, p->rope, nwg, qkv_bytes);
        }
        if (!fsh.ok) {
            const double bytes = (double)(m.n_past + 1) * m.Egqa * 4.0 + m.E * 9.0;
            if (cx.want(GGML_HIP_KCLASS_ATTN, bytes)) {
                Timed tm(GGML_HIP_KCLASS_ATTN, bytes);
                long long *ts_attn = cx.next_ts();
                if (!long_ctx) {
                    launch_attn_decode(p, il, 1, attn_decode_rows(m.C, 1, m.H), f16d, nullptr, ts_attn);
                } else {
                    AttnSplitOneArgs oa = split_attn_args(p, il);
                    AttnSplitArgs &sa = oa.a;
                    sa.sc = p->att_sc; sa.pmax = p->att_pmax; sa.part = p->att_part;
                    const dim3 grid((unsigned)m.H, (unsigned)sa.S);
                    if (attn_one_ok(m, p->att_S)) {
                        launch_attn_split_one(p, oa, f16d);
                    } else {
                        hipLaunchKernelGGL(k_attn_split_scores, grid, dim3(1024), 0, g.stream, sa);
                        hipLaunchKernelGGL(k_attn_split_vp, grid, dim3(1024), attn_split_chunk_max(m.C, sa.S) * 2, g.stream, sa);
                        with_bool(f16d, [&](auto F16D) { hipLaunchKernelGGL(k_attn_split_out<CT(F16D)>, dim3((unsigned)m.H), dim3(256), 0, g.stream, sa); });
                    }
                }
                HIP_CHECK(hipGetLastError());
            }
        }
        if (!fuse_wo) {
            DecMmvqArgs a;
            memset(&a, 0, sizeof(a));
            a.w[0] = w.wo; a.x = actE; a.nb = nbE; a.dst = p->xb; a.res = xin;
            matvec(1, epi_add, x_q8, x_q8, a, nullptr, nullptr, (int)((E + 7) / 8), wo_bytes);
        }
        if (!fuse_x) rmsq(p->xb, ln.ffn_norm, nullptr);
        {
            DecMmvqArgs a;
            memset(&a, 0, sizeof(a));
            a.w[0] = w.w1; a.w[1] = w.w3; a.x = actE; a.xf = p->xb; a.xw = ln.ffn_norm; a.eps = m.eps; a.nb = nbE;
            a.dst = p->gate;
            matvec(2, epi_gate, x_norm, x_norm, a, nullptr, nullptr, (int)((F + 7) / 8), 2.0 * F * nbE * bb + nbE * 40.0 + F * 4.0);
        }
        if (!fuse_x)
            cx.other((double)F * 5.25, [&] {
                with_bool(f16d, [&](auto F16D) {
                    hipLaunchKernelGGL(k_quant_row<CT(F16D)>, grid1(nbF * 32), dim3(256), 0, g.stream, (const float *)p->gate,
                                       (int)nbF, p->f_lo, p->f_hi, p->f_d, p->f_s);
                });
            });
        {
            DecMmvqArgs a;
            memset(&a, 0, sizeof(a));
            a.w[0] = w.w2; a.x = actF; a.xf = p->gate; a.nb = nbF; a.dst = xout; a.res = p->xb;
            matvec(3, epi_add, x_f32, x_f32, a, nullptr, nullptr, (int)((E + 7) / 8), (double)E * nbF * bb + nbF * 40.0 + E * 8.0);
        }
    }
    if (!m.output) return;
    const ResultDst dst = plan_result_dst(p);
    if (!big) rmsq(p->xa, p->norm, dst.emb);
    {
        DecMmvqArgs a;
        memset(&a, 0, sizeof(a));
        a.w[0] = p->output; a.x = actE; a.nb = nbE; a.dst = (float *)dst.logits;
        a.xf = p->xa; a.xw = p->norm; a.eps = m.eps;
        matvec(4, epi_store, x_norm, x_q8, a, dst.emb, nullptr, (int)((m.V + 7) / 8), (double)m.V * nbE * bb + nbE * 40.0 + m.V * 4.0);
    }
}

static void launch_mmvq_kn(int nseg, const KWeight *const *ws, float *const *dsts, const KAct &x, int N, const float *res) {
    const KWeight &w = *ws[0];
    const int64_t K = w.nsb * 256, nsb = w.nsb;
    int64_t Mt = 0;
    for (int i = 0; i < nseg; i++) Mt += ws[i]->M;
    const size_t col_lds = (size_t)K + (size_t)nsb * (4 + 64);
    for (int c0 = 0; c0 < N;) {
        int ncols = 8;
        while (ncols > 1 && (ncols > N - c0 || (size_t)ncols * col_lds > 150 * 1024)) ncols >>= 1;
        const size_t lds = (size_t)ncols * col_lds;
        const int per_cu = (int)std::max<size_t>(1, std::min<size_t>(8, (150 * 1024) / std::max<size_t>(lds, 1)));
        const int nwg = (int)std::min<int64_t>((Mt + 3) / 4, (int64_t)g.num_cus * per_cu);
        MmvqKArgs a;
        memset(&a, 0, sizeof(a));
        a.w = w;
        a.x.q8 = x.q8 + (int64_t)c0 * K;
        a.x.d8 = x.d8 + (int64_t)c0 * nsb;
        a.x.bs = x.bs + (int64_t)c0 * nsb * 16;
        a.dst = dsts[0] + (int64_t)c0 * ws[0]->M;
        a.ldd = ws[0]->M;
        a.res = res ? res + (int64_t)c0 * ws[0]->M : nullptr;
        a.nseg = nseg;
        if (nseg > 1) { a.wb = *ws[1]; a.dst_b = dsts[1] + (int64_t)c0 * ws[1]->M; a.ldd_b = ws[1]->M; }
        if (nseg > 2) { a.wc = *ws[2]; a.dst_c = dsts[2] + (int64_t)c0 * ws[2]->M; a.ldd_c = ws[2]->M; }
        with_kt(w.kt, [&](auto KT) { launch_mmvq_k_c<CT(KT)>(a, ncols, nwg, lds); });
        HIP_CHECK(hipGetLastError());
        c0 += ncols;
    }
}
struct RowSrc {
    int xsrc;
    const float *xf, *xw;
    float eps;
    float *y_out;
};
// ... 291 lines not shown
```

### llm_amd/csrc/plan_run.inc

```
template <class F>
static void capture_into(hipGraph_t *graph, hipGraphExec_t *exec, F &&launch) {
    HIP_CHECK(hipStreamBeginCapture(g.stream, hipStreamCaptureModeThreadLocal));
    launch();
    HIP_CHECK(hipStreamEndCapture(g.stream, graph));
    HIP_CHECK(hipGraphInstantiate(exec, *graph, nullptr, nullptr, 0));
}
static bool emb_row_mirrored(const DecodePlan *p) {
    const LlamaMatch &m = p->m;
    return m.embedding && m.embedding->data && p->emb_out && (size_t)m.N * (size_t)m.E * 4 <= ((size_t)128 << 10);
}
static void queue_results(const DecodePlan *p) {
    const LlamaMatch &m = p->m;
    if (m.N == 1 && !m.prompt) g.stat_result_copies += (m.logits && m.logits->backend == GGML_BACKEND_CPU ? 1 : 0) + (emb_row_mirrored(p) ? 1 : 0);
    if (m.logits && m.logits->backend == GGML_BACKEND_CPU) d2h_queue(m.logits->data, p->logits_out, (size_t)m.V * m.N * 4);
    if (emb_row_mirrored(p)) d2h_queue(m.embedding->data, (const char *)p->emb_out, (size_t)m.N * (size_t)m.E * 4);
}
static void token_results_queue(DecodePlan *p) {
    if (p->m.N != 1 || p->m.prompt || !p->ferr) return;
    g.ferr_plan = p;
}
static void tail_deliver(const Backend::TailWait &tw) {
    DecodePlan *tp = (DecodePlan *)tw.plan;
    const char *sl = tp->slot[tw.q];
    if (tw.logits_dst) memcpy(tw.logits_dst, sl, (size_t)tp->m.V * 4);
    if (tw.emb_dst) memcpy(tw.emb_dst, sl + tp->slot_emb_off, (size_t)tp->m.E * 4);
    if (g.spec.pending && g.spec.plan == tw.plan && g.spec.parity == (tw.q ^ 1)) {
        g.spec.fed_id = *(const int32_t *)(sl + tp->slot_id_off);
        g.spec.fed_id_valid = true;
    }
}
static void token_finish(bool can_rerun = true) {
    const Backend::TailWait tw = g.tail;
    g.tail = Backend::TailWait{};
    if (tw.plan) {
        HIP_CHECK(hipEventSynchronize(((DecodePlan *)tw.plan)->slot_ev[tw.q]));
        if (!stg.pending.empty()) d2h_finish();
        else if (tw.staged) stg.small_off = 0;
    } else {
        d2h_finish();
    }
    DecodePlan *p = (DecodePlan *)g.ferr_plan;
    g.ferr_plan = nullptr;
    if (!p || !g.ferr_pin || !*(volatile unsigned *)g.ferr_pin) {
        if (tw.plan) tail_deliver(tw);
        return;
    }
    spec_cancel();
    *(volatile unsigned *)g.ferr_pin = 0;
    g.stat_fused_timeouts++;
    static const char *what =
        "an attention workgroup of k_qkv_attn / k_attn_split_one gave up waiting for rows of its own launch (these launches "
        "need all their workgroups resident at once: is another process, or a CU mask, holding compute units of this GPU?)";
    bool live = false;
    for (auto *q : g_plans) live = live || q == p;
    if (!live) die("%s", what);
    const bool whole = p->m.wte && p->m.output;
    if (!g.opt_fused_fallback || !can_rerun || !whole || p->m.N != 1)
        die("%s; set GGML_HIP_FUSE_ATTN=0 GGML_HIP_ATTN_ONE=0 to run the two-launch forms", what);
    static bool warned = false;
    if (!warned) fprintf(stderr, "libggml_hip: %s — re-running the token on the two-launch forms and keeping them on this device slot\n", what);
    warned = true;
    if (g.opt_fuse_attn || g.opt_attn_one) {
        g.fused_saved_fuse_attn = g.opt_fuse_attn;
        g.fused_saved_attn_one = g.opt_attn_one;
    }
    g.fused_rearm_stretch = g.fused_rearm_stretch ? g.fused_rearm_stretch * 2 : (uint64_t)std::max(0, g.opt_fused_rearm_tokens);
    g.fused_rearm_at = g.opt_fused_rearm_tokens > 0 ? g.stat_plan_tokens + g.fused_rearm_stretch : 0;
    g.opt_fuse_attn = 0;
    g.opt_attn_one = 0;
    if (!g.opt_test_fused_timeout) g.opt_affine = 0;
    g.opt_test_fused_timeout = 0;
    for (auto *q : g_plans) drop_plan_graphs(q);
    const LlamaMatch &m = p->m;
    {
        DecParams hp;
        memset(&hp, 0, sizeof(hp));
        hp.n_past = m.n_past;
        hp.token = m.embd ? ((const int32_t *)m.embd->data)[0] : 0;
        hp.tokens[0] = hp.token;
        h2d_small((char *)p->prm, &hp, sizeof(hp));
        g.stat_result_copies++;
        p->prm_ahead = false;
    }
    plan_launch_decode(p, attn_variant(m, p, m.n_past + 1));
    g.res_plan = nullptr;
    queue_results(p);
    d2h_finish();
    if (*(volatile unsigned *)g.ferr_pin) die("%s — and again on the re-run", what);
}
void finish_pending() {
    if (!g.pending_wait) return;
    const uint64_t t = now_ns();
    g.pending_wait = false;
    token_finish();
    g.ns_wait += now_ns() - t;
}

struct PrepMatch {
    ggml_cgraph *gr = nullptr;
    LlamaMatch m;
    DecodePlan *p = nullptr;
    uint64_t arena_seq = 0, wgen = 0;
    int opt_gen = 0;
};
static bool prepare_decode_plan(ggml_cgraph *gr) {
    if (!g.prep) g.prep = new PrepMatch();
    PrepMatch *pm = (PrepMatch *)g.prep;
    pm->gr = nullptr;
    if (!g.opt_plan || !g.opt_prepare || !gr) return false;
    LlamaMatch m;
    if (!match_llama_decode(gr, m) || m.prompt || m.N != 1 || !plan_weights_resident(m)) return false;
    const std::vector<uint64_t> sig = plan_signature(m);
    const uint64_t wgen = g_dev_wgen[g.device & 63].load(std::memory_order_acquire);
    DecodePlan *p = nullptr;
    for (auto *q : g_plans)
        if (q->sig == sig && q->wgen == wgen) p = q;
    if (!p) return false;
    pm->m = m;
    pm->p = p;
    pm->arena_seq = g_arena_seq.load(std::memory_order_acquire);
    pm->wgen = wgen;
    pm->opt_gen = g.opt_gen;
    pm->gr = gr;
    return true;
}

static DecodePlan *find_or_build_plan(const LlamaMatch &m, const std::vector<uint64_t> &sig, bool batch = false) {
    const uint64_t wgen = g_dev_wgen[g.device & 63].load(std::memory_order_acquire);
    {
        bool stale = false;
        for (auto *q : g_plans) stale = stale || q->wgen != wgen;
        if (stale) drop_all_plans();
    }
    DecodePlan *p = nullptr;
    for (auto *q : g_plans)
        if (q->sig == sig) p = q;
    if (!p) {
        if (g_plans.size() >= 32) drop_all_plans();
        p = build_plan(m, sig, batch);
        p->wgen = wgen;
        g_plans.push_back(p);
    } else {
        p->m = m;
    }
    return p;
}

static void tail_slots(DecodePlan *p) {
    if (p->slot[0]) return;
    p->slot_emb_off = ((size_t)p->m.V * 4 + 255) & ~(size_t)255;
    p->slot_id_off = p->slot_emb_off + (((size_t)p->m.E * 4 + 255) & ~(size_t)255);
    for (int q = 0; q < 2; q++) {
        HIP_CHECK(hipHostMalloc((void **)&p->slot[q], p->slot_id_off + 256, hipHostMallocDefault));
        HIP_CHECK(hipEventCreateWithFlags(&p->slot_ev[q], hipEventDisableTiming));
    }
}
static bool try_decode_plan(ggml_cgraph *gr, bool defer_wait = false) {
    g.chain_plan = nullptr;
    const bool greedy_next = g.greedy_hint;
    g.greedy_hint = false;
    if (!g.opt_plan) return false;
    if (g.fused_rearm_at && g.stat_plan_tokens >= g.fused_rearm_at) {
        g.fused_rearm_at = 0;
        g.opt_fuse_attn = g.fused_saved_fuse_attn;
        g.opt_attn_one = g.fused_saved_attn_one;
        g.stat_fused_rearms++;
        spec_cancel();
        if (g.stream) HIP_CHECK(hipStreamSynchronize(g.stream));
        for (auto *q : g_plans) drop_plan_graphs(q);
    }
    const uint64_t t0 = now_ns();
    LlamaMatch m;
    DecodePlan *p = nullptr;
    if (PrepMatch *pm = (PrepMatch *)g.prep) {
        if (pm->gr == gr && pm->arena_seq == g_arena_seq.load(std::memory_order_acquire) && pm->opt_gen == g.opt_gen &&
            pm->wgen == g_dev_wgen[g.device & 63].load(std::memory_order_acquire))
            for (auto *q : g_plans)
                if (q == pm->p) p = q;
        if (p) {
            m = pm->m;
            p->m = m;
            g.stat_prepared_tokens++;
        }
        pm->gr = nullptr;
    }
    if (!p) {
        if (!match_llama_decode(gr, m)) return false;
        if (!plan_weights_resident(m)) {
            upload_inputs(gr);
            if (!plan_weights_resident(m)) return false;
        }
        if (m.prompt && m.kquant && !k_prompt_weights(m, nullptr)) {
            if (m.N > MULTI_MAX_N) return false;
            LlamaMatch m2;
            tl_k_prompt_off = true;
            const bool ok = match_llama_decode(gr, m2);
            tl_k_prompt_off = false;
            if (!ok) return false;
            m = m2;
        }
        p = find_or_build_plan(m, plan_signature(m));
    }
    const uint64_t t1 = now_ns();
    bool spec_hit = false;
    int hit_q = 0;
    if (g.spec.pending) {
        g.spec.pending = false;
        const bool same = g.spec.plan == (void *)p && m.N == 1 && !m.prompt && m.embd && m.n_past == g.spec.n_past &&
                          attn_variant(m, p, m.n_past + 1) == g.spec.av && g.opt_graph && !g.timing.on;
        spec_hit = same && g.spec.fed_id_valid && g.spec.fed_id == ((const int32_t *)m.embd->data)[0];
        hit_q = g.spec.parity;
        if (spec_hit) {
            if (g.opt_speculate_next) g.stat_spec_hits++;
        } else {
            if (g.opt_speculate_next) g.stat_spec_misses++;
            g.spec.cooldown = 8;
            spec_take_back();
        }
        (spec_hit ? g.stat_tail_hits : g.stat_tail_misses)++;
    }
    if (!spec_hit) res_settle();
    DecParams hp;
    hp.n_past = m.n_past;
    hp.token = m.embd ? ((const int32_t *)m.embd->data)[0] : 0;
    hp.store_at = hp.pad1 = 0;
    for (int i = 0; i < 32; i++) {
        hp.tokens[i] = (m.embd && i < m.N && !m.prompt) ? ((const int32_t *)m.embd->data)[i] : 0;
        if (m.wte && (hp.tokens[i] < 0 || hp.tokens[i] >= m.wte->ne[1])) die("token id %d out of range", hp.tokens[i]);
    }
    if (!spec_hit) {
        h2d_small((char *)p->prm, &hp, sizeof(hp));
        p->prm_ahead = false;
        if (m.N == 1 && !m.prompt) g.stat_result_copies++;
    }
    if (m.prompt) {
        if (m.wte) {
            const int32_t *ids = (const int32_t *)m.embd->data;
            for (int i = 0; i < m.N; i++)
                if (ids[i] < 0 || ids[i] >= m.wte->ne[1]) die("token id %d out of range", ids[i]);
            h2d_small((char *)p->p_tok, ids, (size_t)m.N * 4);
        }
        plan_launch_prompt(p);
        if (m.logits && m.logits->backend == GGML_BACKEND_CPU)
            d2h_queue(m.logits->data, p->logits_out, (size_t)m.V * m.N * 4);
        const uint64_t t2p = now_ns();
        g.ns_match += t1 - t0;
        g.ns_launch += t2p - t1;
        g.stat_prompt_plan_tokens += (uint64_t)m.N;
        if (defer_wait) {
            g.pending_wait = true;
            g.pending_light = true;
            return true;
        }
        d2h_finish();
        g.ns_wait += now_ns() - t2p;
        return true;
    }
    const bool use_graph = g.opt_graph && !g.timing.on;
    {
        const uint64_t dgen = g_dev_gen[g.device & 63].load(std::memory_order_relaxed);
        if (p->dev_gen != dgen) {
            if (p->dev_gen) {
                HIP_CHECK(hipStreamSynchronize(g.stream));
                drop_plan_graphs(p);
            }
            p->dev_gen = dgen;
        }
    }
    const int av = attn_variant(m, p, m.n_past + 1);
    const bool long_ctx = av == AV_SPLIT;
    auto launch = [&] {
        if (m.N > 1 && !m.kquant && !m.f16w)
            plan_launch_multi(p);
        else
            plan_launch_decode(p, av);
    };
    if (g.spec.cooldown > 0) g.spec.cooldown--;
    const bool tail = g.opt_token_tail && (g.opt_speculate_next || greedy_next) && g.spec.cooldown == 0 && use_graph && m.N == 1 && m.logits && m.wte &&
                      m.output && m.embd && p->logits_alt && m.n_past + 2 < m.C;
    const auto launch_tail = [&](int v, int q) {
        VariantGraphs &vg = p->graphs[v];
        if (!vg.tail_exec[q]) {
            tail_slots(p);
            p->out_set = q;
            capture_into(&vg.tail_graph[q], &vg.tail_exec[q], [&] {
                hipLaunchKernelGGL(k_kv_row_save, dim3(kv_row_grid(p)), dim3(256), 0, g.stream, (const DecParams *)p->prm, (const __half *)p->mem_k,
                                   (const __half *)p->mem_v, p->kv_save[q], (int)m.L, (int)m.C, (int)m.Egqa);
                plan_launch_decode(p, v);
                hipLaunchKernelGGL(k_token_tail, dim3(TOKEN_TAIL_WGS), dim3(1024), 0, g.stream, (const float *)p->res_logits(q), (int)m.V,
                                   (size_t)m.E * 4 <= ((size_t)128 << 10) ? (const float *)p->res_emb(q) : (const float *)nullptr, (int)m.E, p->prm, p->slot[q],
                                   (int)p->slot_emb_off, (int)p->slot_id_off);
            });
            p->out_set = 0;
        }
        HIP_CHECK(hipGraphLaunch(vg.tail_exec[q], g.stream));
        HIP_CHECK(hipEventRecord(p->slot_ev[q], g.stream));
        p->prm_ahead = true;
    };
    int tail_q = -1;
    if (spec_hit) {
        tail_q = hit_q;
        p->replays++;
    } else if (tail) {
        tail_q = 0;
        launch_tail(av, tail_q);
        p->replays++;
    } else if (use_graph) {
        VariantGraphs &vg = p->graphs[av];
        if (!vg.exec) capture_into(&vg.graph, &vg.exec, launch);
        HIP_CHECK(hipGraphLaunch(vg.exec, g.stream));
        p->replays++;
    } else {
        launch();
    }
    if (tail_q >= 0) {
        g.stat_tail_tokens++;
        g.tail.plan = p;
        g.tail.q = tail_q;
        g.tail.logits_dst = m.logits->backend == GGML_BACKEND_CPU ? m.logits->data : nullptr;
        g.tail.emb_dst = emb_row_mirrored(p) ? m.embedding->data : nullptr;
        g.tail.staged = !spec_hit;
        p->cur_set = tail_q;
        g.res_plan = p;
    } else {
        queue_results(p);
    }
    token_results_queue(p);
    if (tail) {
        const int av2 = attn_variant(m, p, m.n_past + 2);
        launch_tail(av2, tail_q ^ 1);
        g.spec.pending = true;
        g.spec.plan = p;
        g.spec.n_past = m.n_past + 1;
        g.spec.av = av2;
        g.spec.parity = tail_q ^ 1;
        g.spec.fed_id_valid = false;
    }
    const uint64_t t2 = now_ns();
    g.ns_match += t1 - t0;
    g.ns_launch += t2 - t1;
    g.stat_plan_tokens += (uint64_t)m.N;
    if (long_ctx) g.stat_split_tokens++;
    if (m.N == 1 && !long_ctx) {
        const FusedShape fs = fused_qkv_shape(m, av_heads_split(av));
        if (fs.ok) g.stat_fused_tokens++;
        if (fs.ok && fs.wo) g.stat_fused_wo_tokens++;
        if (fs.ok && fs.affine) g.stat_fused_affine_tokens++;
    }
    if (av >= AV_FUSED2) g.stat_fused_heads_tokens++;
    if (m.kquant) g.stat_kplan_tokens += (uint64_t)m.N;
    g.chain_plan = (m.N == 1 && m.logits && m.wte) ? (void *)p : nullptr;
    g.chain_graph = gr;
    if (defer_wait) {
        g.pending_wait = true;
        g.pending_light = m.N > 1;
        return true;
    }
    token_finish();
    g.ns_wait += now_ns() - t2;
    return true;
}

static int decode_greedy_chain(ggml_cgraph *last, int n, int32_t *out_tokens, float *last_logits) {
    finish_pending();
    DecodePlan *p = (DecodePlan *)g.chain_plan;
    if (!p || g.chain_graph != last || n < 1) return -1;
    bool live = false;
    for (auto *q : g_plans) live = live || q == p;
    const LlamaMatch &m = p->m;
    if (!live || m.N != 1 || !m.logits || !m.wte || m.n_past + 1 + n > m.C) return -1;
    if (p->prm_ahead) {
        if (!m.embd) return -1;
        DecParams hp;
        memset(&hp, 0, sizeof(hp));
        hp.n_past = m.n_past;
        hp.token = hp.tokens[0] = ((const int32_t *)m.embd->data)[0];
        h2d_small((char *)p->prm, &hp, sizeof(hp));
        p->prm_ahead = false;
    }
    spec_cancel();
    const float *first_logits = (const float *)plan_cur_logits(p);
    g.res_plan = nullptr;
    if (p->chain_cap < n) {
        if (p->chain_out) (void)hipFree(p->chain_out);
        p->chain_cap = std::max(n, 256);
        HIP_CHECK(hipMalloc((void **)&p->chain_out, (size_t)p->chain_cap * 4));
    }
    if (!p->chain_ring) HIP_CHECK(hipMalloc((void **)&p->chain_ring, 64 * 4));
    const bool use_graph = g.opt_graph && !g.timing.on && p->any_captured();
    int i0 = 0;
    if (use_graph && g.opt_chain_k > 1) {
        const int K = g.opt_chain_k;
        if ((const char *)first_logits != p->logits_out) {
            HIP_CHECK(hipMemcpyAsync(p->logits_out, first_logits, (size_t)m.V * 4, hipMemcpyDeviceToDevice, g.stream));
            first_logits = (const float *)p->logits_out;
        }
        const auto long_at = [&](int i) { return attn_variant(m, p, m.n_past + 1 + i + 1) != AV_SHORT; };
        while (i0 + K <= n && !long_at(i0 + K - 1)) {
            if (!p->exec_chain || p->chain_k != K) {
                if (p->exec_chain) (void)hipGraphExecDestroy(p->exec_chain);
                if (p->graph_chain) (void)hipGraphDestroy(p->graph_chain);
                capture_into(&p->graph_chain, &p->exec_chain, [&] {
                    for (int k = 0; k < K; k++) {
                        hipLaunchKernelGGL(k_argmax_next, dim3(1), dim3(1024), 0, g.stream, (const float *)p->logits_out, (int)m.V, p->prm,
                                           p->chain_ring + k);
                        plan_launch_decode(p, AV_SHORT);
                    }
                });
                p->chain_k = K;
            }
            HIP_CHECK(hipGraphLaunch(p->exec_chain, g.stream));
            if (fused_qkv_shape(m).ok) g.stat_fused_tokens += (uint64_t)K;
            HIP_CHECK(hipMemcpyAsync(p->chain_out + i0, p->chain_ring, (size_t)K * 4, hipMemcpyDeviceToDevice, g.stream));
            i0 += K;
        }
    }
    for (int i = i0; i < n; i++) {
        hipLaunchKernelGGL(k_argmax_next, dim3(1), dim3(1024), 0, g.stream, i == 0 ? first_logits : (const float *)p->logits_out, (int)m.V,
                           p->prm, p->chain_out + i);
        const int av = attn_variant(m, p, m.n_past + 1 + i + 1);
        if (av != AV_SPLIT && fused_qkv_shape(m, av_heads_split(av)).ok) g.stat_fused_tokens++;
        if (av >= AV_FUSED2) g.stat_fused_heads_tokens++;
        if (use_graph) {
            VariantGraphs &vg = p->graphs[av];
            if (!vg.exec) capture_into(&vg.graph, &vg.exec, [&] { plan_launch_decode(p, av); });
            if (!vg.exec2) HIP_CHECK(hipGraphInstantiate(&vg.exec2, vg.graph, nullptr, nullptr, 0));
            HIP_CHECK(hipGraphLaunch((i & 1) ? vg.exec2 : vg.exec, g.stream));
        } else {
            plan_launch_decode(p, av);
        }
    }
    HIP_CHECK(hipGetLastError());
    d2h_queue(out_tokens, (const char *)p->chain_out, (size_t)n * 4);
    if (last_logits) d2h_queue(last_logits, p->logits_out, (size_t)m.V * 4);
    token_results_queue(p);
    token_finish(false);
    p->m.n_past += n;
    p->replays += use_graph ? (uint64_t)n : 0;
    g.stat_plan_tokens += (uint64_t)n;
    g.chain_plan = nullptr;
    return 0;
}

constexpr int BATCH_CHAIN_MAX_STEPS = 4096;
static int decode_batch_steps(ggml_cgraph *const *graphs, int B, int n_steps, int32_t *out_ids, bool chain) {
    ensure_init();
    finish_pending();
    spec_cancel();
    g.chain_plan = nullptr;
    res_settle();
    if (PrepMatch *pm = (PrepMatch *)g.prep) pm->gr = nullptr;
    if (!g.opt_plan || !g.opt_plan_batch || (chain && !g.opt_plan_batch_chain)) return -1;
    if (n_steps < 1 || n_steps > BATCH_CHAIN_MAX_STEPS) return -1;
    const uint64_t t0 = now_ns();
    std::vector<LlamaMatch> ms((size_t)B);
    std::vector<uint64_t> sig;
    for (int c = 0; c < B; c++) {
        LlamaMatch &m = ms[(size_t)c];
        if (!match_llama_decode(graphs[c], m)) return -1;
        if (m.N != 1 || m.prompt || m.kquant || !m.wte || !m.output || !m.embd || !m.logits || !m.embedding) return -1;
        if (m.n_past + n_steps > m.C || (qt_of(m.wtype) < 0 && !m.f16w)) return -1;
        for (const ggml_tensor *t : {m.memory_k, m.memory_v}) {
            const DevTensor *e = (const DevTensor *)t->extra;
            if (e && e->magic == 0x48495054 && e->slot != g_cur_slot()) return -1;
        }
    }
    if (attn_decode_lds(ms[0].C, ms[0].D) > ATTN_DECODE_LDS_MAX || (!ms[0].f16w && !multi_shape_ok(ms[0], B))) return -1;
    ws_reset();
    for (int c = 0; c < B; c++) {
        const LlamaMatch &m = ms[(size_t)c];
        if (!plan_weights_resident(m)) {
            upload_inputs(graphs[c]);
            if (!plan_weights_resident(m)) return -1;
        }
        std::vector<uint64_t> s = plan_signature(m, false);
        if (c == 0) sig = std::move(s);
        else if (s != sig) return -1;
    }
    std::vector<__half *> mk((size_t)B), mv((size_t)B);
    for (int c = 0; c < B; c++) {
        mk[(size_t)c] = (__half *)dev_ptr(ms[(size_t)c].memory_k);
        mv[(size_t)c] = (__half *)dev_ptr(ms[(size_t)c].memory_v);
        for (int d = 0; d < c; d++)
// ... 76 lines not shown
```

### llm_amd/csrc/plan_shapes.inc

```

struct F16W {
    const __half *p;
    int64_t ld, M;
};
static const int LAYER_MATS = 7;
template <class W>
struct LayerMats {
    W wq{}, wk{}, wv{}, wo{}, w1{}, w2{}, w3{};
    const W &at(int i) const {
        const W *const all[LAYER_MATS] = {&wq, &wk, &wv, &wo, &w1, &w2, &w3};
        return *all[i];
    }
    W &at(int i) { return const_cast<W &>(static_cast<const LayerMats *>(this)->at(i)); }
};
struct LayerW : LayerMats<const ggml_tensor *> {
    const ggml_tensor *attn_norm = nullptr, *ffn_norm = nullptr;
    const ggml_tensor *cur = nullptr;
    bool k_store = false, v_store = false;
};
static const int PROMPT_PLAN_MAX = 4096;
#define MULTI_MAX_N 31
struct LlamaMatch {
    int L = 0;
    int64_t E = 0, H = 0, Hkv = 0, D = 0, F = 0, V = 0, C = 0, Egqa = 0;
    int n_past = 0, n_dims = 0;
    int N = 1;
    bool prompt = false;
    bool kquant = false;
    bool f16w = false;
    float eps = 0, freq_base = 0, freq_scale = 0, kq_scale = 0;
    ggml_type wtype = GGML_TYPE_F32;
    const ggml_tensor *wte = nullptr, *norm = nullptr, *output = nullptr, *embd = nullptr, *memory_k = nullptr,
                      *memory_v = nullptr;
    ggml_tensor *logits = nullptr, *embedding = nullptr;
    const ggml_tensor *stage_in = nullptr, *stage_out = nullptr;
    std::vector<LayerW> layers;
};
enum { AV_SHORT = 0, AV_SPLIT = 1, AV_FUSED2 = 2, AV_FUSED3 = 3, AV_FUSED4 = 4, AV_COUNT = 5 };
static inline int av_heads_split(int av) { return av >= AV_FUSED2 ? av : 1; }
struct VariantGraphs {
    hipGraph_t graph = nullptr;
    hipGraphExec_t exec = nullptr, exec2 = nullptr;
    hipGraph_t tail_graph[2] = {nullptr, nullptr};
    hipGraphExec_t tail_exec[2] = {nullptr, nullptr};
    void drop() {
        for (hipGraphExec_t e : {exec, exec2, tail_exec[0], tail_exec[1]})
            if (e) (void)hipGraphExecDestroy(e);
        for (hipGraph_t gr : {graph, tail_graph[0], tail_graph[1]})
            if (gr) (void)hipGraphDestroy(gr);
        *this = VariantGraphs{};
    }
};
struct DecodePlan {
    std::vector<uint64_t> sig;
    LlamaMatch m;
    using LW = LayerMats<QWeight>;
    using KLW = LayerMats<KWeight>;
    using FLW = LayerMats<F16W>;
    std::vector<LW> lw;
    std::vector<KLW> klw;
    std::vector<FLW> flw;
    struct LayerNorms {
        const float *attn_norm, *ffn_norm;
    };
    std::vector<LayerNorms> ln;
    F16W f_wte{}, f_output{};
    KWeight k_wte{}, k_output{};
    float *k_kf = nullptr, *k_vf = nullptr, *k_att = nullptr, *k_g3 = nullptr;
    int8_t *k_q8 = nullptr;
    float *k_d8 = nullptr;
    int16_t *k_bs = nullptr;
    QWeight wte, output;
    const float *norm = nullptr;
    __half *mem_k = nullptr, *mem_v = nullptr;
    __half *mem_k_at(int il) const { return mem_k + (size_t)il * m.C * m.Egqa; }
    __half *mem_v_at(int il) const { return mem_v + (size_t)il * m.C * m.Egqa; }
    int64_t kv_off(int il) const { return (int64_t)il * m.C * m.Egqa; }
    bool batch = false;
    BatchCols *bcols = nullptr;
    char *pool = nullptr;
    DecParams *prm = nullptr;
    float *rope = nullptr;
    unsigned *epoch = nullptr;
    const void *hot = nullptr;
    unsigned *ferr = nullptr;
    unsigned long long *gran = nullptr;
    unsigned long long *gran_at(int il) const { return gran + (size_t)il * (size_t)((m.E + 2 * m.Egqa) / 2); }
    unsigned long long *ogran = nullptr;
    unsigned long long *dead_gran = nullptr;
    uint64_t dev_gen = 0;
    uint64_t wgen = 0;
    float *xa = nullptr, *xb = nullptr, *q = nullptr, *gate = nullptr, *logits = nullptr;
    int8_t *e_lo = nullptr, *e_hi = nullptr, *f_lo = nullptr, *f_hi = nullptr;
    float *e_d = nullptr, *f_d = nullptr;
    int *e_s = nullptr, *f_s = nullptr;
    float *e_dT = nullptr, *f_dT = nullptr;
    int *e_sT = nullptr, *f_sT = nullptr;
    float *p_te = nullptr, *p_qf = nullptr, *p_kf = nullptr, *p_vf = nullptr, *p_mg = nullptr, *p_g1 = nullptr, *p_g3 = nullptr, *p_sc = nullptr;
    _Float16 *p_x16 = nullptr, *p_p16 = nullptr;
    int *p_tok = nullptr;
    float *stage_in = nullptr, *stage_out = nullptr;
    float *emb_out = nullptr;
    char *logits_out = nullptr;
    char *logits_alt = nullptr;
    float *emb_alt = nullptr;
    int cur_set = 0;
    int out_set = 0;
    char *res_logits(int q) const { return q ? logits_alt : logits_out; }
    float *res_emb(int q) const { return emb_out ? (q ? emb_alt : emb_out) : nullptr; }
    char *slot[2] = {nullptr, nullptr};
    hipEvent_t slot_ev[2] = {nullptr, nullptr};
    size_t slot_emb_off = 0, slot_id_off = 0;
    __half *kv_save[2] = {nullptr, nullptr};
    bool prm_ahead = false;
    int *chain_out = nullptr;
    int *chain_ring = nullptr;
    int chain_cap = 0;
    VariantGraphs graphs[AV_COUNT];
    bool any_captured() const {
        for (const VariantGraphs &v : graphs)
            if (v.exec) return true;
        return false;
    }
    float *att_sc = nullptr, *att_pmax = nullptr, *att_part = nullptr;
    unsigned long long *att_mxg = nullptr, *att_sumg = nullptr, *att_partg = nullptr;
    unsigned long long *att_mxg_at(int il) const { return att_mxg + (size_t)il * m.H * att_S; }
    unsigned long long *att_sumg_at(int il) const { return att_sumg + (size_t)il * m.H * att_S * 2; }
    unsigned long long *att_partg_at(int il) const { return att_partg + (size_t)il * m.H * att_S * m.D; }
    unsigned *att_cnt = nullptr;
    int att_S = 1;
    hipGraph_t graph_chain = nullptr;
    hipGraphExec_t exec_chain = nullptr;
    int chain_k = 0;
    uint64_t replays = 0;
    uint64_t w16_gen = 0;
};

std::vector<DecodePlan *> g_plans_[GGML_HIP_MAX_BACKENDS];
#define g_plans (g_plans_[g.slot])

void drop_plan_graphs(DecodePlan *p) {
    for (VariantGraphs &v : p->graphs) v.drop();
    if (p->exec_chain) (void)hipGraphExecDestroy(p->exec_chain);
    if (p->graph_chain) (void)hipGraphDestroy(p->graph_chain);
    p->exec_chain = nullptr;
    p->graph_chain = nullptr;
    p->chain_k = 0;
}
void destroy_plan(DecodePlan *p) {
    drop_plan_graphs(p);
    if (p->chain_ring) (void)hipFree(p->chain_ring);
    if (p->chain_out) (void)hipFree(p->chain_out);
    if (p->pool) (void)hipFree(p->pool);
    for (int q = 0; q < 2; q++) {
        if (p->slot[q]) (void)hipHostFree(p->slot[q]);
        if (p->slot_ev[q]) (void)hipEventDestroy(p->slot_ev[q]);
    }
    if (g.res_plan == (void *)p) g.res_plan = nullptr;
    delete p;
}
char *result_dev_ptr(const ggml_tensor *t) {
    char *d = dev_ptr(t);
    DecodePlan *p = (DecodePlan *)g.res_plan;
    if (!p || p->cur_set != 1 || !p->logits_alt) return d;
    const size_t lb = (size_t)p->m.V * 4, eb = (size_t)p->m.E * 4;
    if (p->logits_out && d >= p->logits_out && d < p->logits_out + lb) return p->logits_alt + (d - p->logits_out);
    if (p->emb_out && d >= (char *)p->emb_out && d < (char *)p->emb_out + eb) return (char *)p->emb_alt + (d - (char *)p->emb_out);
    return d;
}
static void res_settle() {
    DecodePlan *p = nullptr;
    for (auto *q : g_plans)
        if ((void *)q == g.res_plan) p = q;
    g.res_plan = nullptr;
    if (!p || p->cur_set != 1 || !p->logits_alt || !p->logits_out) return;
    HIP_CHECK(hipMemcpyAsync(p->logits_out, p->logits_alt, (size_t)p->m.V * 4, hipMemcpyDeviceToDevice, g.stream));
    if (p->emb_out) HIP_CHECK(hipMemcpyAsync(p->emb_out, p->emb_alt, (size_t)p->m.E * 4, hipMemcpyDeviceToDevice, g.stream));
    p->cur_set = 0;
}
static inline char *plan_cur_logits(const DecodePlan *p) { return p->res_logits(g.res_plan == (const void *)p ? p->cur_set : 0); }
static inline int kv_row_grid(const DecodePlan *p) { return (int)std::min<int64_t>(256, ((int64_t)p->m.L * p->m.Egqa + 255) / 256); }
static void spec_take_back() {
    DecodePlan *p = nullptr;
    for (auto *q : g_plans)
        if ((void *)q == g.spec.plan) p = q;
    if (!p || !p->kv_save[g.spec.parity] || !p->mem_k) return;
    hipLaunchKernelGGL(k_kv_row_restore, dim3(kv_row_grid(p)), dim3(256), 0, g.stream, g.spec.n_past, p->mem_k, p->mem_v,
                       (const __half *)p->kv_save[g.spec.parity], (int)p->m.L, (int)p->m.C, (int)p->m.Egqa);
    HIP_CHECK(hipGetLastError());
}
void spec_cancel() {
    if (!g.spec.pending) return;
    g.spec.pending = false;
    spec_take_back();
    if (g.stream) HIP_CHECK(hipStreamSynchronize(g.stream));
}
void spec_guard_read(const char *d, size_t n) {
    if (!g.spec.pending) return;
    DecodePlan *p = nullptr;
    for (auto *q : g_plans)
        if ((void *)q == g.spec.plan) p = q;
    if (!p || !p->mem_k) return;
    const size_t kvb = (size_t)p->m.L * p->m.C * p->m.Egqa * 2;
    const char *k = (const char *)p->mem_k, *v = (const char *)p->mem_v;
    if ((d < k + kvb && k < d + n) || (d < v + kvb && v < d + n)) spec_cancel();
}
void finish_pending();
void drop_all_plans() {
    finish_pending();
    spec_cancel();
    if (g_plans.empty()) return;
    if (g.stream) HIP_CHECK(hipStreamSynchronize(g.stream));
    for (auto *p : g_plans) destroy_plan(p);
    g_plans.clear();
    g.ferr_plan = nullptr;
}
static inline size_t attn_decode_lds(int64_t C, int64_t D) { return (size_t)(C + D) * 4 + (size_t)C * 2; }
static const size_t ATTN_DECODE_LDS_MAX = 150 * 1024;
static int big_waves(int64_t units, int G, int min_waves) {
    static const int forced = getenv("GGML_HIP_BIG_WAVES") ? atoi(getenv("GGML_HIP_BIG_WAVES")) : 0;
    if (forced >= 8 && forced <= BIG_W) return std::max(forced, min_waves);
    auto score = [&](int W) {
        const int64_t per_round = (int64_t)G * W, rounds = (units + per_round - 1) / per_round;
        return (double)units / (double)(rounds * per_round) * (1.0 - 0.015 * (BIG_W - W));
    };
    int best = BIG_W;
    for (int W = BIG_W - 1; W >= std::max(8, min_waves); W--)
        if (score(W) > score(best) + 1e-9) best = W;
    return best;
}
static int big_min_waves(int xsrc, int epi, int64_t nb) {
    int min_waves = 8;
    if (xsrc == XSRC_Q8) min_waves = (int)((nb + 63) / 64);
    if (xsrc == XSRC_F32) min_waves = (int)((nb * 32 + 24 * 64 - 1) / (24 * 64));
    if (xsrc == XSRC_NORM) min_waves = epi == EPI_QKV ? 10 : 8;
    return std::max(min_waves, 8);
}
static inline int big_groups(int64_t units, int cus) { return (int)std::min<int64_t>(cus, std::max<int64_t>(1, (units + BIG_W - 1) / BIG_W)); }
static inline int64_t big_rounds(int64_t units, int G, int W) { return (units + (int64_t)G * W - 1) / ((int64_t)G * W); }
struct BigShape {
    bool ok;
    int G, W;
    size_t lds;
};
static BigShape big_shape(int xsrc, int epi, int64_t nb, int64_t units) {
    BigShape s;
    s.G = big_groups(units, g.num_cus);
    s.W = big_waves(units, s.G, big_min_waves(xsrc, epi, nb));
    s.ok = big_rounds(units, s.G, s.W) <= 64;
    s.lds = (size_t)((nb + 63) / 64 * 64) * 40;
    return s;
}
struct FusedShape {
    bool ok = false;
    int G = 0, W = 0, S = 1;
    bool wo = false;
    bool affine = false;
};
static FusedShape fused_qkv_shape(const LlamaMatch &m, int S = 1) {
    FusedShape s;
    if (!g.opt_fuse_attn || !g.opt_big || m.kquant || m.f16w || m.N != 1 || m.D > 128 || m.D % 32 != 0) return s;
    const int H = (int)m.H * S;
    const int64_t units = (m.E + 2 * m.Egqa) / 2;
    if (H + 1 > g.num_cus) return s;
    if (device_sharers() > 1 && (int64_t)device_sharers() * H > g.num_cus / 4) return s;
    s.S = S;
// ... 125 lines not shown
```

### llm_amd/ggml.py

```python
import ctypes as C
import os

import numpy as np

_HERE = os.path.dirname(os.path.abspath(__file__))
LIB_PATH = os.environ.get("GGML_HIP_LIB") or os.path.join(_HERE, "libggml_hip.so")

TYPE_F32, TYPE_F16, TYPE_Q4_0, TYPE_Q4_1, TYPE_Q5_0, TYPE_Q5_1, TYPE_Q8_0, TYPE_Q8_1 = 0, 1, 2, 3, 6, 7, 8, 9
TYPE_Q2_K, TYPE_Q3_K, TYPE_Q4_K, TYPE_Q5_K, TYPE_Q6_K, TYPE_Q8_K = 10, 11, 12, 13, 14, 15
TYPE_I8, TYPE_I16, TYPE_I32 = 16, 17, 18
BACKEND_CPU, BACKEND_GPU, BACKEND_GPU_SPLIT = 0, 10, 20
OP_NONE, OP_MUL_MAT = 0, 21
MAX_NODES, MAX_SRC, MAX_NAME, HASHTABLE = 4096, 6, 48, 8273
KCLASS_MMVQ, KCLASS_MMQ_MFMA, KCLASS_ATTN, KCLASS_OTHER = 0, 1, 2, 3
COMM_ID_BYTES = 128
KKIND_BASE = 16

TYPE_NAMES = {TYPE_F32: "f32", TYPE_F16: "f16", TYPE_Q4_0: "q4_0", TYPE_Q4_1: "q4_1", TYPE_Q5_0: "q5_0",
              TYPE_Q5_1: "q5_1", TYPE_Q8_0: "q8_0", TYPE_Q2_K: "q2_K", TYPE_Q3_K: "q3_K", TYPE_Q4_K: "q4_K", TYPE_Q5_K: "q5_K",
              TYPE_Q6_K: "q6_K", TYPE_I32: "i32"}
BLOCK_BYTES = {TYPE_F32: 4, TYPE_F16: 2, TYPE_Q4_0: 18, TYPE_Q4_1: 20, TYPE_Q5_0: 22, TYPE_Q5_1: 24, TYPE_Q8_0: 34,
               TYPE_Q8_1: 40, TYPE_Q2_K: 84, TYPE_Q3_K: 110, TYPE_Q4_K: 144, TYPE_Q5_K: 176, TYPE_Q6_K: 210, TYPE_Q8_K: 292,
               TYPE_I8: 1, TYPE_I16: 2, TYPE_I32: 4}
BLOCK_ELEMS = {TYPE_F32: 1, TYPE_F16: 1, TYPE_Q4_0: 32, TYPE_Q4_1: 32, TYPE_Q5_0: 32, TYPE_Q5_1: 32, TYPE_Q8_0: 32,
# ... 81 lines not shown
    "ggml_is_permuted": (C.c_bool, [TP]),
    "ggml_tensor_overhead": (C.c_size_t, []),
    "ggml_get_data": (C.c_void_p, [TP]),
    "ggml_get_data_f32": (C.c_void_p, [TP]),
    "ggml_get_name": (C.c_char_p, [TP]),
    "ggml_set_name": (TP, [TP, C.c_char_p]),
    "ggml_new_tensor": (TP, [CTX, C.c_int, C.c_int, C.POINTER(C.c_int64)]),
    "ggml_new_tensor_1d": (TP, [CTX, C.c_int, C.c_int64]),
    "ggml_new_tensor_2d": (TP, [CTX, C.c_int, C.c_int64, C.c_int64]),
    "ggml_new_tensor_3d": (TP, [CTX, C.c_int, C.c_int64, C.c_int64, C.c_int64]),
    "ggml_new_tensor_4d": (TP, [CTX, C.c_int, C.c_int64, C.c_int64, C.c_int64, C.c_int64]),
    "ggml_new_i32": (TP, [CTX, C.c_int32]),
    "ggml_new_f32": (TP, [CTX, C.c_float]),
    "ggml_dup_tensor": (TP, [CTX, TP]),
    "ggml_view_tensor": (TP, [CTX, TP]),
    "ggml_dup": (TP, [CTX, TP]),
    "ggml_add": (TP, [CTX, TP, TP]),
    "ggml_add_inplace": (TP, [CTX, TP, TP]),
    "ggml_mul": (TP, [CTX, TP, TP]),
    "ggml_repeat": (TP, [CTX, TP, TP]),
    "ggml_silu": (TP, [CTX, TP]),
    "ggml_gelu": (TP, [CTX, TP]),
    "ggml_norm": (TP, [CTX, TP]),
    "ggml_rms_norm": (TP, [CTX, TP, C.c_float]),
    "ggml_mul_mat": (TP, [CTX, TP, TP]),
    "ggml_scale": (TP, [CTX, TP, TP]),
    "ggml_scale_inplace": (TP, [CTX, TP, TP]),
    "ggml_cpy": (TP, [CTX, TP, TP]),
    "ggml_cont": (TP, [CTX, TP]),
    "ggml_reshape": (TP, [CTX, TP, TP]),
    "ggml_reshape_1d": (TP, [CTX, TP, C.c_int64]),
    "ggml_reshape_2d": (TP, [CTX, TP, C.c_int64, C.c_int64]),
    "ggml_reshape_3d": (TP, [CTX, TP, C.c_int64, C.c_int64, C.c_int64]),
    "ggml_view_1d": (TP, [CTX, TP, C.c_int64, C.c_size_t]),
    "ggml_view_2d": (TP, [CTX, TP, C.c_int64, C.c_int64, C.c_size_t, C.c_size_t]),
    "ggml_view_3d": (TP, [CTX, TP, C.c_int64, C.c_int64, C.c_int64, C.c_size_t, C.c_size_t, C.c_size_t]),
    "ggml_permute": (TP, [CTX, TP, C.c_int, C.c_int, C.c_int, C.c_int]),
    "ggml_transpose": (TP, [CTX, TP]),
    "ggml_get_rows": (TP, [CTX, TP, TP]),
    "ggml_diag_mask_inf": (TP, [CTX, TP, C.c_int]),
    "ggml_diag_mask_inf_inplace": (TP, [CTX, TP, C.c_int]),
    "ggml_soft_max": (TP, [CTX, TP]),
    "ggml_soft_max_inplace": (TP, [CTX, TP]),
    "ggml_rope": (TP, [CTX, TP, C.c_int, C.c_int, C.c_int, C.c_int]),
    "ggml_rope_inplace": (TP, [CTX, TP, C.c_int, C.c_int, C.c_int, C.c_int]),
    "ggml_rope_custom_inplace": (TP, [CTX, TP, C.c_int, C.c_int, C.c_int, C.c_int, C.c_float, C.c_float]),
    "ggml_alibi": (TP, [CTX, TP, C.c_int, C.c_int, C.c_float]),
    "ggml_flash_attn": (TP, [CTX, TP, TP, TP, C.c_bool]),
    "ggml_map_unary_f32": (TP, [CTX, TP, C.c_void_p]),
    "ggml_map_binary_f32": (TP, [CTX, TP, TP, C.c_void_p]),
    "ggml_new_graph": (GP, [CTX]),
    "ggml_graph_overhead": (C.c_size_t, []),
    "ggml_build_forward_expand": (None, [GP, TP]),
    "ggml_build_forward": (ggml_cgraph, [TP]),
    "ggml_graph_plan": (ggml_cplan, [GP, C.c_int]),
    "ggml_graph_compute": (C.c_int, [GP, C.POINTER(ggml_cplan)]),
    "ggml_graph_reset": (None, [GP]),
    "ggml_quantize_q4_0": (C.c_size_t, [C.c_void_p, C.c_void_p, C.c_int, C.c_int, C.c_void_p]),
    "ggml_quantize_q4_1": (C.c_size_t, [C.c_void_p, C.c_void_p, C.c_int, C.c_int, C.c_void_p]),
    "ggml_quantize_q5_0": (C.c_size_t, [C.c_void_p, C.c_void_p, C.c_int, C.c_int, C.c_void_p]),
    "ggml_quantize_q5_1": (C.c_size_t, [C.c_void_p, C.c_void_p, C.c_int, C.c_int, C.c_void_p]),
    "ggml_quantize_q8_0": (C.c_size_t, [C.c_void_p, C.c_void_p, C.c_int, C.c_int, C.c_void_p]),
    "ggml_quantize_q2_K": (C.c_size_t, [C.c_void_p, C.c_void_p, C.c_int, C.c_int, C.c_void_p]),
    "ggml_quantize_q3_K": (C.c_size_t, [C.c_void_p, C.c_void_p, C.c_int, C.c_int, C.c_void_p]),
    "ggml_quantize_q4_K": (C.c_size_t, [C.c_void_p, C.c_void_p, C.c_int, C.c_int, C.c_void_p]),
    "ggml_quantize_q5_K": (C.c_size_t, [C.c_void_p, C.c_void_p, C.c_int, C.c_int, C.c_void_p]),
    "ggml_quantize_q6_K": (C.c_size_t, [C.c_void_p, C.c_void_p, C.c_int, C.c_int, C.c_void_p]),
    "ggml_quantize_chunk": (C.c_size_t, [C.c_int, C.c_void_p, C.c_void_p, C.c_int, C.c_int, C.c_void_p]),
    "ggml_internal_get_type_traits": (ggml_type_traits_t, [C.c_int]),
    "ggml_cpu_has_blas": (C.c_int, []),
    "ggml_cpu_has_gpublas": (C.c_int, []),
}
_HOOKS = {
    "init_XXblas": (None, []),
    "PFX_set_tensor_split": (None, [C.c_void_p]),
    "PFX_mul": (None, [TP, TP, TP]),
    "PFX_can_mul_mat": (C.c_bool, [TP, TP, TP]),
    "PFX_mul_mat_get_wsize": (C.c_size_t, [TP, TP, TP]),
    "PFX_mul_mat": (None, [TP, TP, TP, C.c_void_p, C.c_size_t]),
    "PFX_host_malloc": (C.c_void_p, [C.c_size_t]),
    "PFX_host_free": (None, [C.c_void_p]),
    "PFX_transform_tensor": (None, [C.c_void_p, TP]),
    "PFX_free_data": (None, [TP]),
    "PFX_assign_buffers": (None, [TP]),
    "PFX_assign_buffers_no_scratch": (None, [TP]),
    "PFX_assign_buffers_force_inplace": (None, [TP]),
    "PFX_set_main_device": (None, [C.c_int]),
    "PFX_set_mul_mat_q": (None, [C.c_bool]),
    "PFX_set_scratch_size": (None, [C.c_size_t]),
    "PFX_free_scratch": (None, []),
    "PFX_compute_forward": (C.c_bool, [C.POINTER(ggml_compute_params), TP]),
}
for _k, _v in _HOOKS.items():
    if _k == "init_XXblas":
        PROTOTYPES["ggml_init_hipblas"] = _v
        PROTOTYPES["ggml_init_cublas"] = _v
    else:
        PROTOTYPES[_k.replace("PFX", "ggml_hip")] = _v
        PROTOTYPES[_k.replace("PFX", "ggml_cuda")] = _v
PROTOTYPES.update({
    "ggml_hip_device_count": (C.c_int, []),
    "ggml_hip_slot_physical_device": (C.c_int, [C.c_int]),
    "ggml_hip_thread_session_slot": (C.c_int, []),
    "ggml_hip_synchronize": (None, []),
    "ggml_hip_tensor_get": (None, [TP, C.c_void_p, C.c_size_t, C.c_size_t]),
    "ggml_hip_tensor_set": (None, [TP, C.c_void_p, C.c_size_t, C.c_size_t]),
    "ggml_hip_tensor_device_ptr": (C.c_void_p, [TP]),
    "ggml_hip_memcpy": (None, [C.c_void_p, C.c_void_p, C.c_size_t, C.c_int]),
    "ggml_hip_timing_begin": (None, []),
    "ggml_hip_timing_end": (None, []),
    "ggml_hip_timing_query": (None, [C.c_int, C.POINTER(C.c_double), C.POINTER(C.c_int64), C.POINTER(C.c_double)]),
    "ggml_hip_set_option": (None, [C.c_char_p, C.c_int]),
    "ggml_hip_get_option": (C.c_int, [C.c_char_p]),
    "ggml_hip_get_stat": (C.c_int64, [C.c_char_p]),
    "ggml_hip_read_timeline": (C.c_size_t, [C.c_void_p, C.c_size_t]),
    "ggml_hip_get_main_device": (C.c_int, []),
    "ggml_hip_bind_thread_device": (None, [C.c_int]),
    "ggml_hip_thread_pinned_device": (C.c_int, []),
    "ggml_hip_unbind_thread_device": (None, []),
    "ggml_hip_get_tensor_split": (C.c_int, [C.c_void_p, C.c_int]),
    "ggml_hip_set_layer_split": (None, [C.c_void_p, C.c_int]),
    "ggml_hip_get_layer_split": (C.c_int, [C.c_void_p, C.c_int]),
    "ggml_hip_copy_between_devices": (None, [C.c_int, C.c_void_p, C.c_int, C.c_void_p, C.c_size_t]),
    "ggml_hip_share_stream": (C.c_int, [C.c_int, C.c_int]),
    "ggml_hip_debug_prompt_attention": (C.c_int, [C.c_void_p, C.c_void_p, C.c_void_p, C.c_void_p, C.c_int, C.c_int, C.c_int, C.c_int,
                                                  C.c_int, C.c_int64, C.c_float, C.c_int]),
    "ggml_hip_debug_prompt_attention_plan": (C.c_int, [C.c_void_p, C.c_void_p, C.c_void_p, C.c_void_p, C.c_void_p, C.c_void_p, C.c_void_p,
                                                       C.c_int, C.c_int, C.c_int, C.c_int, C.c_int, C.c_int64, C.c_float, C.c_int]),
    "ggml_hip_debug_mul_mat_cols": (C.c_int, [C.c_void_p, C.c_void_p, C.c_void_p, C.c_int]),
    "ggml_hip_debug_mat_vec_big": (C.c_int, [C.c_void_p, C.c_void_p, C.c_void_p, C.c_int, C.c_int, C.c_void_p, C.c_void_p, C.c_float,
                                             C.c_void_p, C.c_void_p, C.c_void_p, C.c_int, C.c_int, C.c_float, C.c_float, C.c_int64,
                                             C.c_void_p, C.c_void_p]),
    "ggml_hip_debug_mat_vec_kbig": (C.c_int, [C.c_void_p, C.c_void_p, C.c_void_p, C.c_int, C.c_int, C.c_void_p, C.c_void_p, C.c_float,
                                              C.c_void_p, C.c_void_p, C.c_void_p, C.c_int, C.c_int, C.c_float, C.c_float, C.c_int64,
                                              C.c_void_p, C.c_void_p]),
    "ggml_hip_debug_mat_vec_f16": (C.c_int, [C.c_void_p, C.c_void_p, C.c_void_p, C.c_int, C.c_int, C.c_void_p, C.c_void_p, C.c_float,
                                             C.c_void_p, C.c_void_p, C.c_void_p, C.c_int, C.c_int, C.c_float, C.c_float, C.c_int64,
                                             C.c_void_p, C.c_void_p, C.c_int]),
    "ggml_hip_debug_exp_le0": (C.c_int, [C.c_void_p, C.c_void_p]),
    "ggml_hip_decode_greedy_chain": (C.c_int, [C.c_void_p, C.c_int, C.c_void_p, C.c_void_p]),
    "ggml_hip_decode_batch": (C.c_int, [C.c_void_p, C.c_int]),
    "ggml_hip_decode_batch_greedy": (C.c_int, [C.c_void_p, C.c_int, C.c_int, C.c_void_p]),
    "ggml_hip_debug_batch_tail": (C.c_int, [C.c_void_p, C.c_int, C.c_int, C.c_void_p, C.c_void_p, C.c_void_p, C.c_void_p, C.c_void_p]),
    "ggml_hip_topk": (C.c_int, [C.c_void_p, C.c_int64, C.c_int, C.c_void_p, C.c_int, C.c_void_p, C.c_void_p]),
    "ggml_hip_row_probs": (C.c_int, [C.c_void_p, C.c_int64, C.c_int64, C.c_void_p, C.c_void_p]),
    "ggml_hip_quantize": (C.c_size_t, [C.c_int, C.c_void_p, C.c_void_p, C.c_int64, C.c_int64, C.c_void_p]),
    "ggml_hip_quantize_resident": (C.c_int, [C.c_void_p, C.c_void_p, C.c_void_p]),
    "ggml_hip_graph_compute_begin": (C.c_int, [C.c_void_p]),
    "ggml_hip_graph_prepare": (C.c_int, [C.c_void_p]),
    "ggml_hip_graph_compute_end": (None, []),
    "ggml_hip_expect_greedy_next": (None, []),
    "ggml_hip_debug_token_tail": (C.c_int, [C.c_void_p, C.c_int, C.c_void_p, C.c_int, C.c_int, C.c_int, C.c_void_p, C.c_void_p,
                                            C.c_void_p, C.c_void_p, C.c_void_p]),
    "ggml_hip_bench_plan_class": (C.c_int, [C.c_int, C.c_int, C.POINTER(C.c_double), C.POINTER(C.c_int64),
                                            C.POINTER(C.c_double)]),
    "ggml_hip_comm_unique_id": (C.c_int, [C.c_void_p]),
    "ggml_hip_comm_init": (C.c_int, [C.c_int, C.c_int, C.c_void_p]),
    "ggml_hip_comm_destroy": (None, []),
    "ggml_hip_comm_ranks": (C.c_int, []),
    "ggml_hip_comm_send": (None, [C.c_void_p, C.c_size_t, C.c_int]),
    "ggml_hip_comm_recv": (None, [C.c_void_p, C.c_size_t, C.c_int]),
    "ggml_hip_comm_sendrecv": (None, [C.c_void_p, C.c_int, C.c_void_p, C.c_int, C.c_size_t]),
    "ggml_hip_bench_empty": (C.c_int, [C.c_int, C.c_int, C.c_int, C.c_int, C.c_int, C.c_int, C.POINTER(C.c_double)]),
    "ggml_hip_version": (C.c_char_p, []),
})

_lib = None


def lib():
    global _lib
    if _lib is None:
        if not os.path.exists(LIB_PATH):
            raise RuntimeError(
                f"{LIB_PATH} is missing: run `python -c 'import __graft_entry__ as g; g.build()'` "
                "(hipcc --offload-arch=gfx950). There is no CPU / pure-Python fallback for the compute path.")
        L = C.CDLL(LIB_PATH)
        for name, (res, args) in PROTOTYPES.items():
            f = getattr(L, name)
            f.restype = res
            f.argtypes = args
        _lib = L
    return _lib


def has_gpu():
    try:
        return lib().ggml_hip_device_count() > 0
    except Exception:
        return False


def row_bytes(t, k):
    return k // BLOCK_ELEMS[t] * BLOCK_BYTES[t]


def quantize(t, x):
    x = np.ascontiguousarray(x, dtype=np.float32)
    if t == TYPE_F32:
        return x.view(np.uint8).reshape(-1).copy()
    if t == TYPE_F16:
        out = np.zeros(x.size, dtype=np.uint16)
        lib().ggml_fp32_to_fp16_row(x.ctypes.data, out.ctypes.data, x.size)
        return out.view(np.uint8)
    k = x.shape[-1]
    out = np.zeros(row_bytes(t, x.size), dtype=np.uint8)
    hist = np.zeros(16, dtype=np.int64)
    fn = getattr(lib(), "ggml_quantize_" + TYPE_NAMES[t])
    got = fn(x.ctypes.data, out.ctypes.data, x.size, k, hist.ctypes.data)
    assert got == out.size, (got, out.size)
    return out


def quantize_on_device(t, x):
    x = np.ascontiguousarray(x, dtype=np.float32)
    out = np.zeros(row_bytes(t, x.size), dtype=np.uint8)
    hist = np.zeros(16, dtype=np.int64)
    got = lib().ggml_hip_quantize(t, x.ctypes.data, out.ctypes.data, x.size, x.shape[-1], hist.ctypes.data)
    assert got == out.size, (got, out.size)
    return out, hist


def topk(tensor, row, k, extra_ids=()):
    extra = np.ascontiguousarray(extra_ids, dtype=np.int32)
    vals = np.zeros(k + extra.size, dtype=np.float32)
    ids = np.zeros(k + extra.size, dtype=np.int32)
    ptr = tensor.ptr if isinstance(tensor, Tensor) else tensor
    rc = lib().ggml_hip_topk(ptr, row, k, extra.ctypes.data if extra.size else None, extra.size, vals.ctypes.data, ids.ctypes.data)
    if rc != 0:
        raise ValueError("ggml_hip_topk: bad arguments")
    return vals, ids


def row_probs(node, targets, row_begin=0):
    targets = np.ascontiguousarray(targets, dtype=np.int32)
    out = np.zeros(targets.size, dtype=np.float32)
    ptr = node.ptr if isinstance(node, Tensor) else node
    rc = lib().ggml_hip_row_probs(ptr, row_begin, targets.size, targets.ctypes.data if targets.size else None, out.ctypes.data)
    if rc != 0:
        raise ValueError("ggml_hip_row_probs: bad arguments")
    return out


class Tensor:

    def __init__(self, ptr, ctx):
        assert bool(ptr), "Should not be null"
        self.ptr = ptr
        self.ctx = ctx

    @property
    def t(self):
        return self.ptr.contents

    @property
    def ne(self):
        return tuple(self.t.ne)

    @property
    def nb(self):
        return tuple(self.t.nb)

    def nbytes(self):
        return lib().ggml_nbytes(self.ptr)

    def nelements(self):
        return lib().ggml_nelements(self.ptr)

    def set_name(self, name):
        lib().ggml_set_name(self.ptr, name.encode())
        return self

    def name(self):
        return lib().ggml_get_name(self.ptr).decode()

    def write_data(self, arr):
        arr = np.ascontiguousarray(arr)
        assert arr.nbytes <= self.nbytes(), (arr.nbytes, self.nbytes())
        C.memmove(self.t.data, arr.ctypes.data, arr.nbytes)
        return self

    def read_data(self, dtype=np.float32, count=None):
        n = self.nbytes() if count is None else count * np.dtype(dtype).itemsize
        buf = (C.c_char * n).from_address(self.t.data)
        return np.frombuffer(buf, dtype=dtype).copy()

    def device_get(self, dtype=np.float32):
        out = np.zeros(self.nbytes() // np.dtype(dtype).itemsize, dtype=dtype)
        lib().ggml_hip_tensor_get(self.ptr, out.ctypes.data, 0, out.nbytes)
        return out

    def transfer_to_gpu(self):
        self.t.backend = BACKEND_GPU
        lib().ggml_hip_transform_tensor(self.t.data, self.ptr)
        self.ctx._offloaded.append(self)
        return self

    def offload(self):
        lib().ggml_hip_assign_buffers(self.ptr)
        return self

    def offload_no_scratch(self):
        lib().ggml_hip_assign_buffers_no_scratch(self.ptr)
        self.ctx._offloaded.append(self)
        return self

# ... 130 lines not shown
```

Baseline: 862.1.

## Fold next-token embedding, rope table and KV row save into token tail kernel

The token tail kernel, which copies logits and picks the argmax, now also does work for the speculative next step when enabled. Block 0 dequantizes the embedding row of the chosen token into a new xnext buffer, one extra block builds the rope table and bumps the epoch, and extra blocks save the KV row at the next position. The pre-captured next-step graph then skips its separate k_get_rows_q, k_rope_table and k_kv_row_save launches. This removes several small kernel launches per decoded token, at the cost of a second set of captured tail graphs, a larger tail grid, and extra position bookkeeping in DecParams.

```diff
diff --git a/include/ggml_hip.h b/include/ggml_hip.h
--- a/include/ggml_hip.h
+++ b/include/ggml_hip.h
@@ -483,6 +483,12 @@
 GGML_API int ggml_hip_debug_exp_le0(uint16_t *out_fast, uint16_t *out_ref);
 GGML_API int ggml_hip_debug_token_tail(const float *logits, int V, const float *emb, int E, int n_past, int misalign,
                                        int32_t *id_tail, int32_t *id_argmax, float *slot_logits, float *slot_emb, int32_t *prm_out);
+GGML_API int ggml_hip_debug_token_tail_prepare(const float *logits, int V, const void *wte_raw, int wtype, int E, int n_past,
+                                               uint32_t epoch_in, int parity, int zeroed, int L, int C, int Egqa,
+                                               const uint16_t *mem_k, const uint16_t *mem_v, float theta_scale, float freq_scale,
+                                               int half_d, int32_t *id_out, int32_t *prm_out, float *row, float *table,
+                                               uint32_t *epoch_out, uint16_t *save, float *row_ref, float *table_ref,
+                                               uint32_t *epoch_ref, uint16_t *save_ref);
 GGML_API int ggml_hip_debug_batch_tail(const float *logits, int B, int V, const int32_t *pos_in, const int32_t *tokens_in,
                                        int32_t *ids_out, int32_t *prm_out, int32_t *pos_out);
 GGML_API int ggml_hip_debug_mul_mat_cols(const struct ggml_tensor *w, const float *x, float *out, int N);
diff --git a/llm_amd/csrc/backend_state.inc b/llm_amd/csrc/backend_state.inc
--- a/llm_amd/csrc/backend_state.inc
+++ b/llm_amd/csrc/backend_state.inc
@@ -93,13 +93,14 @@
     ggml_cgraph *chain_graph = nullptr;
     bool pending_wait = false;
     bool pending_light = false;
-    int opt_speculate_next = 0, opt_token_tail = 1;
+    int opt_speculate_next = 0, opt_token_tail = 1, opt_tail_prepare = 1;
     bool greedy_hint = false;
     struct Spec {
         bool pending = false;
         void *plan = nullptr;
         int n_past = 0, av = 0;
         int parity = 0;
+        bool prepared = false;
         int32_t fed_id = 0;
         bool fed_id_valid = false;
         int cooldown = 0;
@@ -112,7 +113,7 @@
     } tail;
     void *res_plan = nullptr;
     uint64_t stat_tail_tokens = 0, stat_result_copies = 0, stat_tail_hits = 0, stat_tail_misses = 0;
-    uint64_t stat_spec_hits = 0, stat_spec_misses = 0;
+    uint64_t stat_spec_hits = 0, stat_spec_misses = 0, stat_tail_prepared_tokens = 0;
     unsigned *ferr_pin = nullptr;
     void *ferr_plan = nullptr;
     int opt_fused_fallback = 1, opt_fused_rearm_tokens = 256;
@@ -162,6 +163,7 @@
     {"prepare", &Backend::opt_prepare, OPT_ENV},
     {"speculate_next", &Backend::opt_speculate_next, OPT_ENV, FX_SPECULATE_NEXT},
     {"token_tail", &Backend::opt_token_tail, OPT_ENV, FX_SPECULATE_NEXT},
+    {"tail_prepare", &Backend::opt_tail_prepare, OPT_ENV | OPT_DROPS},
     {"fuse_attn", &Backend::opt_fuse_attn, OPT_ENV | OPT_DROPS, FX_FUSE_ATTN},
     {"fuse_wo", &Backend::opt_fuse_wo, OPT_ENV | OPT_DROPS},
     {"warm_mb", &Backend::opt_warm_mb, OPT_ENV | OPT_DROPS},
@@ -221,6 +223,7 @@
     {"tail_tokens", &Backend::stat_tail_tokens},
     {"tail_hits", &Backend::stat_tail_hits},
     {"tail_misses", &Backend::stat_tail_misses},
+    {"tail_prepared_tokens", &Backend::stat_tail_prepared_tokens},
     {"result_copies", &Backend::stat_result_copies},
     {"generic_graphs", &Backend::stat_generic_graphs},
     {"alibi_fused", &Backend::stat_alibi_fused},
diff --git a/llm_amd/csrc/backend_tools.inc b/llm_amd/csrc/backend_tools.inc
--- a/llm_amd/csrc/backend_tools.inc
+++ b/llm_amd/csrc/backend_tools.inc
@@ -534,7 +534,7 @@
     HIP_CHECK(hipMemcpy(pb, &hp, sizeof(hp), hipMemcpyHostToDevice));
     hipLaunchKernelGGL(k_argmax_next, dim3(1), dim3(1024), 0, g.stream, (const float *)dl, V, pa, ida);
     hipLaunchKernelGGL(k_token_tail, dim3(TOKEN_TAIL_WGS), dim3(1024), 0, g.stream, (const float *)dl, V, emb ? (const float *)de : (const float *)nullptr,
-                       E, pb, slot, (int)emb_off, (int)id_off);
+                       E, pb, slot, (int)emb_off, (int)id_off, TailPrep{});
     HIP_CHECK(hipGetLastError());
     HIP_CHECK(hipStreamSynchronize(g.stream));
     HIP_CHECK(hipMemcpy(id_argmax, ida, 4, hipMemcpyDeviceToHost));
@@ -547,6 +547,90 @@
     if (emb && slot_emb) memcpy(slot_emb, slot + emb_off, (size_t)E * 4);
     HIP_CHECK(hipHostFree(slot));
     HIP_CHECK(hipFree(d));
+    return 0;
+}
+
+int ggml_hip_debug_token_tail_prepare(const float *logits, int V, const void *wte_raw, int wtype, int E, int n_past, uint32_t epoch_in,
+                                      int parity, int zeroed, int L, int C, int Egqa, const uint16_t *mem_k, const uint16_t *mem_v,
+                                      float theta_scale, float freq_scale, int half_d, int32_t *id_out, int32_t *prm_out, float *row,
+                                      float *table, uint32_t *epoch_out, uint16_t *save, float *row_ref, float *table_ref,
+                                      uint32_t *epoch_ref, uint16_t *save_ref) {
+    const int qt = qt_of((ggml_type)wtype);
+    if (!logits || V < 1 || !wte_raw || qt < 0 || E < 32 || E % 32 || n_past < 0 || n_past + 1 >= C || (parity & ~1) || L < 1 || Egqa < 1 ||
+        !mem_k || !mem_v || half_d < 1 || half_d > 64 || !id_out || !prm_out || !row || !table || !epoch_out || !save || !row_ref ||
+        !table_ref || !epoch_ref || !save_ref)
+        return -1;
+    SlotLock lk;
+    ensure_init();
+    finish_pending();
+    std::vector<char *> owned;
+    const int64_t nb = E / 32;
+    const size_t raw_bytes = (size_t)V * nb * (size_t)blk_bytes(qt), nkv = (size_t)L * C * Egqa * 2, nsave = (size_t)L * Egqa * 4;
+    char *draw = debug_buf(raw_bytes, wte_raw, owned);
+    size_t off[5];
+    char *dsoa = debug_buf(qw_layout(qt, V, nb, off), nullptr, owned);
+    relayout_launch(draw, qt, V, nb, dsoa);
+    const QWeight w = qw_at(dsoa, qt, V, nb);
+    char *dl = debug_buf((size_t)V * 4, logits, owned);
+    char *dk = debug_buf(nkv, mem_k, owned), *dv = debug_buf(nkv, mem_v, owned);
+    DecParams hp;
+    memset(&hp, 0, sizeof(hp));
+    hp.n_past = hp.pos_tail[0] = hp.pos_tail[1] = n_past;
+    DecParams *prm[2];
+    unsigned *ep[2];
+    char *drow[2], *dtab[2], *dsave[2];
+    for (int i = 0; i < 2; i++) {
+        prm[i] = (DecParams *)debug_buf(sizeof(hp), &hp, owned);
+        ep[i] = (unsigned *)debug_buf(4, &epoch_in, owned);
+        drow[i] = debug_buf((size_t)E * 4, nullptr, owned);
+        dtab[i] = debug_buf(128 * 4, nullptr, owned);
+        dsave[i] = debug_buf(nsave, nullptr, owned);
+    }
+    int *ida = (int *)debug_buf(4, nullptr, owned);
+    char *slot = nullptr;
+    const size_t id_off = ((size_t)V * 4 + 255) & ~(size_t)255;
+    HIP_CHECK(hipHostMalloc((void **)&slot, id_off + 256, hipHostMallocDefault));
+    memset(slot, 0xff, id_off + 256);
+    TailPrep tp;
+    memset(&tp, 0, sizeof(tp));
+    if (!zeroed) {
+        tp.xnext = (float *)drow[0];
+        tp.wte = w;
+        tp.rope = (float *)dtab[0]; tp.epoch = ep[0];
+        tp.theta_scale = theta_scale; tp.freq_scale = freq_scale; tp.half_d = half_d;
+        tp.mem_k = (const __half *)dk; tp.mem_v = (const __half *)dv; tp.save = (__half *)dsave[0];
+        tp.L = L; tp.C = C; tp.Egqa = Egqa;
+        tp.pos_in = &prm[0]->pos_tail[parity]; tp.pos_out = &prm[0]->pos_tail[parity ^ 1];
+    }
+    hipLaunchKernelGGL(k_token_tail, dim3(token_tail_grid(!zeroed, (long)L * Egqa)), dim3(1024), 0, g.stream, (const float *)dl, V,
+                       (const float *)nullptr, 0, prm[0], slot, (int)id_off, (int)id_off, tp);
+    hipLaunchKernelGGL(k_argmax_next, dim3(1), dim3(1024), 0, g.stream, (const float *)dl, V, prm[1], ida);
+    hipLaunchKernelGGL(k_kv_row_save, dim3((unsigned)std::min<int64_t>(256, ((int64_t)L * Egqa + 255) / 256)), dim3(256), 0, g.stream,
+                       (const DecParams *)prm[1], (const __half *)dk, (const __half *)dv, (__half *)dsave[1], L, C, Egqa);
+    hipLaunchKernelGGL(k_get_rows_q, dim3((unsigned)((nb + 255) / 256), 1), dim3(256), 0, g.stream, w, (const int *)&prm[1]->token,
+                       (float *)drow[1], (int64_t)E);
+    hipLaunchKernelGGL(k_rope_table, dim3(1), dim3(128), 0, g.stream, (const DecParams *)prm[1], theta_scale, freq_scale, half_d,
+                       (float *)dtab[1], ep[1]);
+    HIP_CHECK(hipGetLastError());
+    float *rows[2] = {row, row_ref}, *tabs[2] = {table, table_ref};
+    uint32_t *eps[2] = {epoch_out, epoch_ref};
+    uint16_t *saves[2] = {save, save_ref};
+    for (int i = 0; i < 2; i++) {
+        d2h_queue(rows[i], drow[i], (size_t)E * 4);
+        d2h_queue(tabs[i], dtab[i], 128 * 4);
+        d2h_queue(eps[i], (const char *)ep[i], 4);
+        d2h_queue(saves[i], dsave[i], nsave);
+    }
+    d2h_queue(&hp, (const char *)prm[0], sizeof(hp));
+    d2h_finish();
+    prm_out[0] = hp.n_past;
+    prm_out[1] = hp.token;
+    prm_out[2] = hp.tokens[0];
+    prm_out[3] = hp.pos_tail[0];
+    prm_out[4] = hp.pos_tail[1];
+    *id_out = *(const int32_t *)(slot + id_off);
+    HIP_CHECK(hipHostFree(slot));
+    for (char *b : owned) HIP_CHECK(hipFree(b));
     return 0;
 }
 
diff --git a/llm_amd/csrc/kernels/decode.h b/llm_amd/csrc/kernels/decode.h
--- a/llm_amd/csrc/kernels/decode.h
+++ b/llm_amd/csrc/kernels/decode.h
@@ -9,6 +9,7 @@
     int store_at;
     int pad1;
     int tokens[32];
+    int pos_tail[2];
 };
 constexpr int BATCH_COLS_MAX = 8;
 struct BatchCols {
@@ -110,30 +111,114 @@
         mem_v[(il * Egqa + c) * C + pos] = save[n + i];
     }
 }
+struct TailPrep {
+    float *xnext;
+    QWeight wte;
+    float *rope;
+    unsigned *epoch;
+    float theta_scale, freq_scale;
+    int half_d;
+    const __half *mem_k, *mem_v;
+    __half *save;
+    int L, C, Egqa;
+    const int *pos_in;
+    int *pos_out;
+};
 constexpr int TOKEN_TAIL_WGS = 8;
+constexpr int TOKEN_TAIL_SAVE_WGS_MAX = 128;
+static inline int token_tail_grid(bool prep, long n_save) {
+    if (!prep) return TOKEN_TAIL_WGS;
+    const long s = (n_save + 1023) / 1024;
+    return TOKEN_TAIL_WGS + 1 + (int)(s < TOKEN_TAIL_SAVE_WGS_MAX ? s : TOKEN_TAIL_SAVE_WGS_MAX);
+}
+__device__ __forceinline__ void rope_table_pair(int pos, int c, int kk, float theta_scale, float freq_scale, float *__restrict__ out);
+__device__ __forceinline__ void tail_embed_row(const QWeight &w, int64_t row, float *__restrict__ dst) {
+    const int qt = w.qt;
+    const bool has_m = qt == QT_Q4_1 || qt == QT_Q5_1;
+    const bool has_h = qt == QT_Q5_0 || qt == QT_Q5_1;
+    const int zero = qt == QT_Q4_0 ? 8 : qt == QT_Q5_0 ? 16 : 0;
+    for (int64_t e4 = threadIdx.x; e4 < w.nb * 8; e4 += 1024) {
+        const int64_t i = row * w.nb + (e4 >> 3);
+        const int o = (int)(e4 & 7) * 4, j0 = o & 15;
+        const bool up = o >= 16;
+        const float d = __half2float(w.d[i]);
+        float v[4];
+        if (qt == QT_Q8_0) {
+            const int8_t *q = (const int8_t *)((up ? w.qs2 : w.qs) + i * 16 + j0);
+#pragma unroll
+            for (int u = 0; u < 4; u++) v[u] = q[u] * d;
+        } else {
+            const uint8_t *qs = w.qs + i * 16 + j0;
+            const float m = has_m ? __half2float(w.m[i]) : 0.0f;
+            const uint32_t qh = has_h ? w.qh[i] : 0u;
+#pragma unroll
+            for (int u = 0; u < 4; u++) {
+                const int j = j0 + u;
+                const int xh = !has_h ? 0 : up ? (int)((qh >> (j + 12)) & 0x10u) : (int)(((qh >> j) << 4) & 0x10u);
+                const int x = ((up ? (qs[u] >> 4) : (qs[u] & 0x0F)) | xh) - zero;
+                v[u] = has_m ? x * d + m : x * d;
+            }
+        }
+        ((float4 *)dst)[e4] = make_float4(v[0], v[1], v[2], v[3]);
+    }
+}
 __global__ void __launch_bounds__(1024) k_token_tail(const float *__restrict__ logits, int V, const float *__restrict__ emb, int E,
-                                                     DecParams *prm, char *__restrict__ slot, int emb_off, int id_off) {
-    const int gtid = blockIdx.x * 1024 + threadIdx.x, total = gridDim.x * 1024;
-    float *sl = (float *)slot, *se = (float *)(slot + emb_off);
-    if (((uintptr_t)logits & 15) == 0) {
-        const int V4 = V >> 2;
-        for (int i = gtid; i < V4; i += total) ((float4 *)sl)[i] = ((const float4 *)logits)[i];
-        if (gtid < (V & 3)) sl[(V4 << 2) + gtid] = logits[(V4 << 2) + gtid];
-    } else {
-        for (int i = gtid; i < V; i += total) sl[i] = logits[i];
-    }
-    if (emb) {
-        if (((uintptr_t)emb & 15) == 0 && (E & 3) == 0)
-            for (int i = gtid; i < (E >> 2); i += total) ((float4 *)se)[i] = ((const float4 *)emb)[i];
-        else
-            for (int i = gtid; i < E; i += total) se[i] = emb[i];
+                                                     DecParams *prm, char *__restrict__ slot, int emb_off, int id_off, const TailPrep tp) {
+    const bool prep = tp.xnext != nullptr;
+    if ((int)blockIdx.x >= TOKEN_TAIL_WGS) {
+        if (!prep) return;
+        const int pos = *tp.pos_in + 1;
+        if (blockIdx.x == TOKEN_TAIL_WGS) {
+            const int kk = threadIdx.x;
+            if (tp.epoch && kk == 0) {
+                const unsigned e = *tp.epoch + 1u;
+                *tp.epoch = e ? e : 1u;
+            }
+            if (kk < tp.half_d) rope_table_pair(pos, 0, kk, tp.theta_scale, tp.freq_scale, tp.rope);
+            return;
+        }
+        if (!tp.save || pos < 0 || pos >= tp.C) return;
+        const long n = (long)tp.L * tp.Egqa, C = tp.C, nwg = (long)gridDim.x - (TOKEN_TAIL_WGS + 1);
+        for (long i = ((long)blockIdx.x - (TOKEN_TAIL_WGS + 1)) * 1024 + threadIdx.x; i < n; i += nwg * 1024) {
+            const long il = i / tp.Egqa, c = i % tp.Egqa;
+            tp.save[i] = tp.mem_k[(il * C + pos) * tp.Egqa + c];
+            tp.save[n + i] = tp.mem_v[(il * tp.Egqa + c) * C + pos];
+        }
+        return;
+    }
+    const int first = prep ? 1 : 0;
+    if ((int)blockIdx.x >= first) {
+        const int gtid = ((int)blockIdx.x - first) * 1024 + threadIdx.x, total = (TOKEN_TAIL_WGS - first) * 1024;
+        float *sl = (float *)slot, *se = (float *)(slot + emb_off);
+        if (((uintptr_t)logits & 15) == 0) {
+            const int V4 = V >> 2;
+            for (int i = gtid; i < V4; i += total) ((float4 *)sl)[i] = ((const float4 *)logits)[i];
+            if (gtid < (V & 3)) sl[(V4 << 2) + gtid] = logits[(V4 << 2) + gtid];
+        } else {
+            for (int i = gtid; i < V; i += total) sl[i] = logits[i];
+        }
+        if (emb) {
+            if (((uintptr_t)emb & 15) == 0 && (E & 3) == 0)
+                for (int i = gtid; i < (E >> 2); i += total) ((float4 *)se)[i] = ((const float4 *)emb)[i];
+            else
+                for (int i = gtid; i < E; i += total) se[i] = emb[i];
+        }
     }
     if (blockIdx.x != 0) return;
-    const int bi = argmax_first_block(logits, V);
+    __shared__ int s_bi;
+    const int bi0 = argmax_first_block(logits, V);
+    if (threadIdx.x == 0) s_bi = bi0;
+    if (prep) {
+        __syncthreads();
+        const int bi = s_bi;
+        if (bi >= 0 && bi < tp.wte.M) tail_embed_row(tp.wte, bi, tp.xnext);
+    }
     if (threadIdx.x == 0) {
+        const int bi = bi0, pos = prm->n_past + 1;
         prm->token = bi;
         prm->tokens[0] = bi;
-        prm->n_past = prm->n_past + 1;
+        prm->n_past = pos;
+        if (prep) *tp.pos_out = pos;
         *(int *)(slot + id_off) = bi;
     }
 }
diff --git a/llm_amd/csrc/plan_build.inc b/llm_amd/csrc/plan_build.inc
--- a/llm_amd/csrc/plan_build.inc
+++ b/llm_amd/csrc/plan_build.inc
@@ -175,6 +175,7 @@
     c.take(p->emb_alt, spec ? E * 4 : 0);
     c.take(p->kv_save[0], spec ? (size_t)m.L * m.Egqa * 4 : 0);
     c.take(p->kv_save[1], spec ? (size_t)m.L * m.Egqa * 4 : 0);
+    c.take(p->xnext, spec && m.wte && !kq && !m.f16w ? E * 4 : 0);
     c.take(p->epoch, 256);
     const size_t units = (size_t)((m.E + 2 * m.Egqa) / 2);
     c.take(p->gran, one ? (size_t)m.L * units * 8 : 0);
diff --git a/llm_amd/csrc/plan_decode.inc b/llm_amd/csrc/plan_decode.inc
--- a/llm_amd/csrc/plan_decode.inc
+++ b/llm_amd/csrc/plan_decode.inc
@@ -218,14 +218,15 @@
     constexpr std::integral_constant<int, XSRC_NORM> x_norm{};
     constexpr std::integral_constant<int, XSRC_Q8> x_q8{};
     constexpr std::integral_constant<int, XSRC_F32> x_f32{};
-    if (m.wte)
+    const bool prepared = p->open_prepared;
+    if (m.wte && !prepared)
         cx.other((double)E * 4.6, [&] {
             hipLaunchKernelGGL(k_get_rows_q, dim3((unsigned)((nbE + 255) / 256), 1), dim3(256), 0, g.stream, p->wte,
                                (const int *)&p->prm->token, p->xa, E);
         });
     const FusedShape fsh = long_ctx ? FusedShape{} : fused_qkv_shape(m, av_heads_split(av));
     const bool rope_for_fused = fsh.ok && (cx.mask & (1u << GGML_HIP_KCLASS_MMVQ)) && (cx.kind_mask & 1u) && !(cx.mask & (1u << GGML_HIP_KCLASS_OTHER));
-    if (big && (cx.want(GGML_HIP_KCLASS_OTHER, (double)m.D * 4.0) || rope_for_fused)) {
+    if (big && !prepared && (cx.want(GGML_HIP_KCLASS_OTHER, (double)m.D * 4.0) || rope_for_fused)) {
         hipLaunchKernelGGL(k_rope_table, dim3(1), dim3(128), 0, g.stream, (const DecParams *)p->prm, theta_scale,
                            m.freq_scale, (int)(m.D >> 1), p->rope, p->epoch);
         HIP_CHECK(hipGetLastError());
@@ -237,7 +238,7 @@
         const int wl = (same_layer && cx.kind_mask != ~0u) ? 0 : il;
         const DecodePlan::LW &w = p->lw[wl];
         const DecodePlan::LayerNorms &ln = p->ln[wl];
-        float *const xin = (il == 0 && !m.wte) ? p->stage_in : p->xa;
+        float *const xin = il != 0 ? p->xa : !m.wte ? p->stage_in : prepared ? p->xnext : p->xa;
         float *const xout = (il == m.L - 1 && !m.output) ? p->stage_out : p->xa;
         if (!fuse_x) rmsq(xin, ln.attn_norm, nullptr);
         {
diff --git a/llm_amd/csrc/plan_run.inc b/llm_amd/csrc/plan_run.inc
--- a/llm_amd/csrc/plan_run.inc
+++ b/llm_amd/csrc/plan_run.inc
@@ -155,6 +155,24 @@
         HIP_CHECK(hipEventCreateWithFlags(&p->slot_ev[q], hipEventDisableTiming));
     }
 }
+static bool tail_prepares(const DecodePlan *p) {
+    const LlamaMatch &m = p->m;
+    return g.opt_tail_prepare && g.opt_big && !m.kquant && !m.f16w && m.N == 1 && m.wte && m.output && qt_of(m.wtype) >= 0 && p->xnext && p->kv_save[0] && p->mem_k &&
+           p->mem_v && m.D / 2 <= 64 && m.E % 32 == 0;
+}
+static TailPrep tail_prep_args(const DecodePlan *p, int q) {
+    const LlamaMatch &m = p->m;
+    TailPrep tp;
+    memset(&tp, 0, sizeof(tp));
+    tp.xnext = p->xnext;
+    tp.wte = p->wte;
+    tp.rope = p->rope; tp.epoch = p->epoch;
+    tp.theta_scale = powf(m.freq_base, -2.0f / m.n_dims); tp.freq_scale = m.freq_scale; tp.half_d = (int)(m.D >> 1);
+    tp.mem_k = p->mem_k; tp.mem_v = p->mem_v; tp.save = p->kv_save[q ^ 1];
+    tp.L = m.L; tp.C = (int)m.C; tp.Egqa = (int)m.Egqa;
+    tp.pos_in = &p->prm->pos_tail[q]; tp.pos_out = &p->prm->pos_tail[q ^ 1];
+    return tp;
+}
 static bool try_decode_plan(ggml_cgraph *gr, bool defer_wait = false) {
     g.chain_plan = nullptr;
     const bool greedy_next = g.greedy_hint;
@@ -212,6 +230,7 @@
         hit_q = g.spec.parity;
         if (spec_hit) {
             if (g.opt_speculate_next) g.stat_spec_hits++;
+            if (g.spec.prepared) g.stat_tail_prepared_tokens++;
         } else {
             if (g.opt_speculate_next) g.stat_spec_misses++;
             g.spec.cooldown = 8;
@@ -224,6 +243,7 @@
     hp.n_past = m.n_past;
     hp.token = m.embd ? ((const int32_t *)m.embd->data)[0] : 0;
     hp.store_at = hp.pad1 = 0;
+    hp.pos_tail[0] = hp.pos_tail[1] = m.n_past;
     for (int i = 0; i < 32; i++) {
         hp.tokens[i] = (m.embd && i < m.N && !m.prompt) ? ((const int32_t *)m.embd->data)[i] : 0;
         if (m.wte && (hp.tokens[i] < 0 || hp.tokens[i] >= m.wte->ne[1])) die("token id %d out of range", hp.tokens[i]);
@@ -278,24 +298,31 @@
     if (g.spec.cooldown > 0) g.spec.cooldown--;
     const bool tail = g.opt_token_tail && (g.opt_speculate_next || greedy_next) && g.spec.cooldown == 0 && use_graph && m.N == 1 && m.logits && m.wte &&
                       m.output && m.embd && p->logits_alt && m.n_past + 2 < m.C;
-    const auto launch_tail = [&](int v, int q) {
+    const bool prep = tail_prepares(p);
+    const auto launch_tail = [&](int v, int q, bool ahead) {
         VariantGraphs &vg = p->graphs[v];
-        if (!vg.tail_exec[q]) {
+        const int fl = prep && ahead ? TAIL_AHEAD : TAIL_FIRST;
+        if (!vg.tail_exec[fl][q]) {
             tail_slots(p);
             p->out_set = q;
-            capture_into(&vg.tail_graph[q], &vg.tail_exec[q], [&] {
-                hipLaunchKernelGGL(k_kv_row_save, dim3(kv_row_grid(p)), dim3(256), 0, g.stream, (const DecParams *)p->prm, (const __half *)p->mem_k,
-                                   (const __half *)p->mem_v, p->kv_save[q], (int)m.L, (int)m.C, (int)m.Egqa);
+            p->open_prepared = fl == TAIL_AHEAD;
+            capture_into(&vg.tail_graph[fl][q], &vg.tail_exec[fl][q], [&] {
+                if (!prep)
+                    hipLaunchKernelGGL(k_kv_row_save, dim3(kv_row_grid(p)), dim3(256), 0, g.stream, (const DecParams *)p->prm, (const __half *)p->mem_k,
+                                       (const __half *)p->mem_v, p->kv_save[q], (int)m.L, (int)m.C, (int)m.Egqa);
                 plan_launch_decode(p, v);
-                hipLaunchKernelGGL(k_token_tail, dim3(TOKEN_TAIL_WGS), dim3(1024), 0, g.stream, (const float *)p->res_logits(q), (int)m.V,
+                const TailPrep tp = prep ? tail_prep_args(p, q) : TailPrep{};
+                hipLaunchKernelGGL(k_token_tail, dim3(token_tail_grid(prep, (long)m.L * m.Egqa)), dim3(1024), 0, g.stream, (const float *)p->res_logits(q), (int)m.V,
                                    (size_t)m.E * 4 <= ((size_t)128 << 10) ? (const float *)p->res_emb(q) : (const float *)nullptr, (int)m.E, p->prm, p->slot[q],
-                                   (int)p->slot_emb_off, (int)p->slot_id_off);
+                                   (int)p->slot_emb_off, (int)p->slot_id_off, tp);
             });
             p->out_set = 0;
-        }
-        HIP_CHECK(hipGraphLaunch(vg.tail_exec[q], g.stream));
+            p->open_prepared = false;
+        }
+        HIP_CHECK(hipGraphLaunch(vg.tail_exec[fl][q], g.stream));
         HIP_CHECK(hipEventRecord(p->slot_ev[q], g.stream));
         p->prm_ahead = true;
+        return fl;
     };
     int tail_q = -1;
     if (spec_hit) {
@@ -303,7 +330,7 @@
         p->replays++;
     } else if (tail) {
         tail_q = 0;
-        launch_tail(av, tail_q);
+        launch_tail(av, tail_q, false);
         p->replays++;
     } else if (use_graph) {
         VariantGraphs &vg = p->graphs[av];
@@ -328,7 +355,7 @@
     token_results_queue(p);
     if (tail) {
         const int av2 = attn_variant(m, p, m.n_past + 2);
-        launch_tail(av2, tail_q ^ 1);
+        g.spec.prepared = launch_tail(av2, tail_q ^ 1, true) == TAIL_AHEAD;
         g.spec.pending = true;
         g.spec.plan = p;
         g.spec.n_past = m.n_past + 1;
diff --git a/llm_amd/csrc/plan_shapes.inc b/llm_amd/csrc/plan_shapes.inc
--- a/llm_amd/csrc/plan_shapes.inc
+++ b/llm_amd/csrc/plan_shapes.inc
@@ -37,16 +37,17 @@
     std::vector<LayerW> layers;
 };
 enum { AV_SHORT = 0, AV_SPLIT = 1, AV_FUSED2 = 2, AV_FUSED3 = 3, AV_FUSED4 = 4, AV_COUNT = 5 };
+enum { TAIL_FIRST = 0, TAIL_AHEAD = 1 };
 static inline int av_heads_split(int av) { return av >= AV_FUSED2 ? av : 1; }
 struct VariantGraphs {
     hipGraph_t graph = nullptr;
     hipGraphExec_t exec = nullptr, exec2 = nullptr;
-    hipGraph_t tail_graph[2] = {nullptr, nullptr};
-    hipGraphExec_t tail_exec[2] = {nullptr, nullptr};
+    hipGraph_t tail_graph[2][2] = {{nullptr, nullptr}, {nullptr, nullptr}};
+    hipGraphExec_t tail_exec[2][2] = {{nullptr, nullptr}, {nullptr, nullptr}};
     void drop() {
-        for (hipGraphExec_t e : {exec, exec2, tail_exec[0], tail_exec[1]})
+        for (hipGraphExec_t e : {exec, exec2, tail_exec[0][0], tail_exec[0][1], tail_exec[1][0], tail_exec[1][1]})
             if (e) (void)hipGraphExecDestroy(e);
-        for (hipGraph_t gr : {graph, tail_graph[0], tail_graph[1]})
+        for (hipGraph_t gr : {graph, tail_graph[0][0], tail_graph[0][1], tail_graph[1][0], tail_graph[1][1]})
             if (gr) (void)hipGraphDestroy(gr);
         *this = VariantGraphs{};
     }
@@ -112,6 +113,8 @@
     hipEvent_t slot_ev[2] = {nullptr, nullptr};
     size_t slot_emb_off = 0, slot_id_off = 0;
     __half *kv_save[2] = {nullptr, nullptr};
+    float *xnext = nullptr;
+    bool open_prepared = false;
     bool prm_ahead = false;
     int *chain_out = nullptr;
     int *chain_ring = nullptr;
diff --git a/llm_amd/ggml.py b/llm_amd/ggml.py
--- a/llm_amd/ggml.py
+++ b/llm_amd/ggml.py
@@ -257,6 +257,10 @@
     "ggml_hip_expect_greedy_next": (None, []),
     "ggml_hip_debug_token_tail": (C.c_int, [C.c_void_p, C.c_int, C.c_void_p, C.c_int, C.c_int, C.c_int, C.c_void_p, C.c_void_p,
                                             C.c_void_p, C.c_void_p, C.c_void_p]),
+    "ggml_hip_debug_token_tail_prepare": (C.c_int, [C.c_void_p, C.c_int, C.c_void_p, C.c_int, C.c_int, C.c_int, C.c_uint32, C.c_int,
+                                                    C.c_int, C.c_int, C.c_int, C.c_int, C.c_void_p, C.c_void_p, C.c_float, C.c_float,
+                                                    C.c_int, C.c_void_p, C.c_void_p, C.c_void_p, C.c_void_p, C.c_void_p, C.c_void_p,
+                                                    C.c_void_p, C.c_void_p, C.c_void_p, C.c_void_p]),
     "ggml_hip_bench_plan_class": (C.c_int, [C.c_int, C.c_int, C.POINTER(C.c_double), C.POINTER(C.c_int64),
                                             C.POINTER(C.c_double)]),
     "ggml_hip_comm_unique_id": (C.c_int, [C.c_void_p]),
```

Measured after the change: 876.9 (median of 6 runs). 1.02x the previous value.
